# naturerobots/mesh_navigation

Hardware: AMD Instinct MI355X
Metric: plans/sec (Dijkstra makePlan device path incl. computeVectorMap, 1M-vertex mesh) (higher is better)
Workload: dtype f32

## Files before the change

### mesh_navigation_amd/csrc/mnav.hip

```cpp
#include <hip/hip_runtime.h>

#include <algorithm>
#include <array>
#include <atomic>
#include <chrono>
#include <cmath>
#include <cstdio>
#include <cstdlib>
#include <cstring>
#include <functional>
#include <map>
#include <string>
#include <vector>
#include <unordered_map>
#include <unistd.h>

#include "../../include/mnav.h"
#include "mnav_buf.h"
#include "mnav_build.h"
#include "mnav_eval.h"
#include "mnav_options.h"

using namespace mnav;

namespace {

#define MNAV_GLOBAL __attribute__((address_space(1)))
template <class T>
__device__ __forceinline__ MNAV_GLOBAL T* as_global(T* p) { return (MNAV_GLOBAL T*)p; }
template <class T>
__device__ __forceinline__ MNAV_GLOBAL T* as_global(const GPtr<T>& p) { return (MNAV_GLOBAL T*)p.p; }
typedef unsigned int u32x2 __attribute__((ext_vector_type(2)));
typedef unsigned int u32x4 __attribute__((ext_vector_type(4)));

constexpr int kBlock = 256;
constexpr int kChunk = 96;

#include "mnav_band.h"

#include "mnav_tiles.h"

#include "mnav_shard.h"

#include "mnav_finalize.h"

#include "mnav_plan_kernels.h"

#include "mnav_map_kernels.h"

}
#include "mnav_tb.h"
#include "mnav_tb_finalize.h"
#include "mnav_tbv.h"
#include "mnav_walk.h"
#include "mnav_obstacle.h"
#include "mnav_nbhd.h"
#include "mnav_clearance.h"
#include "mnav_locate.h"
#include "mnav_follow.h"
#include "mnav_rollout.h"
#include "mnav_replan.h"
#include "mnav_replan_each.h"
#include "mnav_tb_warm.h"
#include "mnav_graph.h"

struct WalkJob { const float* vecmap; float seed[3]; uint32_t seed_face; float target[3]; uint32_t target_face; };

__global__ __launch_bounds__(64) void k_backtrack(WalkMesh M, WalkInflation L, const WalkJob* __restrict__ jobs, double step_width, uint32_t cap,
                                                  float* __restrict__ pos_out, uint32_t* __restrict__ face_out, int32_t* __restrict__ ctl)
{
  __shared__ uint32_t list[kWalkScratchWords];
  const uint32_t j = blockIdx.x;
  const WalkJob J = jobs[j];
  if (!J.vecmap) { if (threadIdx.x == 0) { ctl[2 * j] = 0; ctl[2 * j + 1] = 0; } return; }
  WalkField Fd;
  Fd.vecmap = J.vecmap;
  for (int k = 0; k < 3; ++k) Fd.seed_vs[k] = M.faces[3 * (size_t)J.seed_face + k];
  uint32_t n = 0;
  const int st = walk_backtrack(M, Fd, L, w3(J.seed[0], J.seed[1], J.seed[2]), J.seed_face, w3(J.target[0], J.target[1], J.target[2]), J.target_face,
                                step_width, cap, pos_out + 3 * (size_t)cap * j, face_out + (size_t)cap * j, &n, list);
  ctl[2 * j] = st; ctl[2 * j + 1] = (int32_t)n;
}
#include "mnav_fleet.h"
#include "mnav_plans.h"
namespace {

struct Slot {
  DevBuf<float> dist, dirn, vecmap;
  DevBuf<PopKey> tkey;
  DevBuf<uint32_t> pred, cutf, stamp, dirty, list0, list1;
  DevBuf<uint32_t> wlist0, wlist1, wstamp;
  Ctl* ctl = nullptr;
  DevBuf<Cnt> cnt;
  bool cvp_ready = false, band_ready = false;
  DevBuf<uint32_t> tpend0, tpend1;
  DevBuf<float> tlast;
  TCtl* tctl = nullptr;
  DevBuf<TCnt> tcnt;
  bool tile_ready = false;
};

}

struct mnav_ctx {
  int device = 0;
  Stream stream;
  std::string err;
  std::atomic<int> cancel{ 0 };
  DevBuf<uint32_t> d_cancel;
  PinnedBuf<uint32_t> h_one;
  Stream cancel_stream;
  uint32_t V = 0, F = 0, E = 0;
  std::vector<float> h_xyz, h_cost;
  std::vector<uint32_t> h_row_ptr, h_nbr_u;
  TbState tb; tb::Args tb_args{};
  bool tb_args_valid = false;
  bool want_vec = false;
  bool resident_vecmap = false;
  std::vector<uint32_t> caller_slot;
  std::vector<uint32_t> h_faces;
  std::vector<uint32_t> h_vf_ptr, h_vf;
  DevBuf<uint32_t> d_faces, d_vf_ptr, d_vf; bool walk_mesh_valid = false;
  DevBuf<float> d_walk_pos; DevBuf<uint32_t> d_walk_face; size_t walk_cap = 0;
  Event ev_link[2];
  DevBuf<WalkJob> d_walk_jobs; DevBuf<int32_t> d_walk_ctl; uint32_t walk_jobs_cap = 0;
  std::vector<uint8_t> h_invalid;
  bool have_mesh = false, have_costs = false, have_normals = false;
  DevBuf<uint32_t> d_row_ptr, d_nbr_u, d_nbr_e, d_crn_ptr, d_edge_vtx;
  DevBuf<CornerIdx> d_crn_idx;
  DevBuf<uint32_t> d_crn_walk;
  DevBuf<float> d_xyz, d_nrm, d_cost, d_w, d_edge_dist;
  DevBuf<uint8_t> d_invalid;
  DevBuf<Nbr> d_nbr; double nbr_limit = NAN; bool nbr_valid = false;
  DevBuf<Corner> d_crn; DevBuf<uint8_t> d_blocked; double crn_limit = NAN; bool crn_valid = false;
  FaceCirculation circ;
  DevBuf<uint32_t> d_verify_any; uint32_t verify_sweeps_used = 0;
  bool cvp_verify = true;
  int walk_max = kKeyWalkMax, descend_max = kDescendWalkMax;
  std::vector<Slot> slots;
  DevBuf<Plan> d_plans; uint32_t plans_cap = 0;
  DevBuf<PlanResult> d_res; PinnedBuf<PlanResult> h_res;
  DevBuf<float*> d_vecptrs;
  DevBuf<uint32_t> d_paths; size_t paths_words = 0; uint32_t path_stride = 0;
  DevBuf<uint32_t> d_over; DevBuf<unsigned long long> d_over_off; DevBuf<uint32_t> d_over_cap;
  DevBuf<uint32_t> d_pack; PinnedBuf<uint32_t> h_pack; DevBuf<uint32_t> d_pack_meta; size_t pack_words = 0, pack_meta_n = 0;
  PinnedBuf<Ctl> h_ctl;
  uint32_t infl_exact_bands = 0;
  DevBuf<float> d_seed_pos; uint32_t seed_pos_cap = 1;
  std::map<uint64_t, GraphExec> graphs;
  int dij_engine = 3;
  int last_engine = 0;
  bool lazy_paths = false;
  bool allow_lazy_paths = true;
  uint32_t max_steps = 1u << 20;
  double max_wall_s = 120.0;
  uint32_t tile_size = 512;
  float rounds_band_mult = 4.0f;
  float tile_band_user = 0.f, tile_band_auto = 1.f;
  DevBuf<uint32_t> d_t_rptr;
  HostTiles tiles_meta;
  DevBuf<uint32_t> d_t_vptr, d_t_verts, d_t_hptr, d_t_halo_verts, d_t_halo_tile, d_t_eptr, d_t_src, d_vert_tile, d_mismatch;
  DevBuf<uint16_t> d_t_rowptr, d_t_col;
  DevBuf<float> d_t_tw; bool tw_valid = false; uint32_t t_nnz = 0;
  struct Shard {
    bool ready = false, active = false, finalized = false;
    uint32_t rank = 0, world = 1, t_lo = 0, t_hi = 0, n_iface = 0, rounds_per_exchange = 8, j = 0;
    uint32_t seed = 0, target = 0; double offset = 0.3; uint32_t goal_tie1 = 0;
    DevBuf<uint32_t> d_iface_vert, d_wake_ptr, d_wake_tile, d_changed, d_minpend;
    DevBuf<uint8_t> d_iface_owner;
    std::vector<uint32_t> iface_vert;
    bool partition = false; DevBuf<uint8_t> d_owned;
    DevBuf<uint32_t> d_walk; uint32_t walk_cap = 0;
    std::map<std::array<uint64_t, 3>, GraphExec> graphs;
  } shard;
  double edge_cost_factor = 0.0;
  struct Layer { DevBuf<float> cost; DevBuf<uint8_t> lethal; DevBuf<float> dist, vec; DevBuf<uint8_t> vstate;
                 bool ready = false, have_vec = false;
                 double inflation_radius = 0, inscribed_radius = 0, inscribed_value = 0, lethal_value = 0; };
  std::vector<Layer> layers;
  DevBuf<Corner> d_crn_infl; bool crn_infl_valid = false;
  DevBuf<uint8_t> d_infl_mask, d_zero_u8;
  DevBuf<float> d_infl_keyd;
  mnav_obs::Bvh obs;
  mnav_nb::State nbhd;
  mnav_clr::State clr;
  mnav_loc::State loc;
  mnav_fol::Staging stage;
  mnav_fol::State fol;
  mnav_fleet::State fleet;
  mnav_fleet::PlanState plans;
  DevBuf<float> d_fnrm; bool have_face_normals = false;
  mnav_rol::Dev rol;
  mnav_chg::Scratch chg;
  mnav_map::State map;
  uint32_t infl_steps = 0, infl_bands = 0; uint64_t infl_evals = 0; float infl_ms = 0.f, infl_ms_wave = 0.f;
  DevBuf<TilePlan> d_tplans; uint32_t tplans_cap = 0;
  PinnedBuf<TCtl> h_tctl;
  size_t tile_lds = 0, fin_lds = 0;
  bool use_graph = true;
  DevBuf<uint32_t> d_wide_prefix; DevBuf<WideSched> d_wide_sched; uint32_t wide_cap = 0;
  DevBuf<float> d_vec3;
  uint32_t wide_groups = 1; Stream stream_g[kWideGroupsMax]; Event ev_fork[kWideGroupsMax];
  uint32_t cvp_wide_min_batch = 32;
  float delta_user = 0.f, delta_auto = 0.f;
  Options opt;
  uint32_t max_steps_auto = 1u << 20;
  DevBuf<uint32_t> d_ring; uint32_t ring_cap = 0; size_t ring_words = 0; PinnedBuf<AsyncCtl> h_actl; DevBuf<uint32_t> d_parked; size_t parked_words = 0;
  struct Replan {
    DevBuf<uint32_t> log; uint32_t len = 0; bool all = false;
    std::vector<uint32_t> seeds, targets, caller_slot; double cost_limit = 1.0, offset = 0.0; bool have_call = false, usable = false;
    bool partial = false;
    bool finalized = false;
    bool slot0_taken = false;
    bool vec_resident = false;
    int each_engines = 0;
    struct Warm {
      DevBuf<uint32_t> d_level; DevBuf<const float*> d_dist; DevBuf<ReplanCnt> d_cnt; uint32_t cap = 0;
      uint32_t plans = 0, kernel = 0, iters = 0, fallback = 0; uint64_t woken = 0, words = 0; bool live = false;
      float ms_warm = 0.f, ms_engine = 0.f, ms_finalize = 0.f;
    } warm;
    DevBuf<uint32_t> d_level, d_old_target; DevBuf<float> d_cut; DevBuf<ReplanCnt> d_cnt; uint32_t cap = 0;
    Event ev[5]; bool have_ev = false;
    uint32_t reason = 0, stat_log_len = 0, tiles_woken = 0, rounds = 0; uint64_t kept = 0, rewound = 0; std::vector<float> levels;
    float ms_level = 0.f, ms_rewind = 0.f, ms_rounds = 0.f, ms_finalize = 0.f;
    struct Each {
      DevBuf<uint8_t> d_cls; DevBuf<float> d_ratio; DevBuf<uint32_t> d_lists, d_counts, d_level;
      DevBuf<Plan> d_plans; DevBuf<TilePlan> d_tplans; DevBuf<float*> d_vecptrs; DevBuf<ReplanCnt> d_cnt; DevBuf<TCtl> d_tctl; DevBuf<PlanResult> d_res;
      uint32_t cap = 0;
      Event ev[7]; bool have_ev = false;
      uint32_t reason = 0, whole_fresh = 0, log_len = 0, counts[3] = { 0, 0, 0 }, tiles_woken = 0, rounds = 0; int fresh_engine = -1;
      uint64_t kept = 0, rewound = 0; std::vector<uint8_t> cls; std::vector<float> levels;
      float ms_classify = 0.f, ms_rewind = 0.f, ms_rounds = 0.f, ms_finalize = 0.f, ms_fresh = 0.f;
    } each;
  } rp;
  uint32_t last_planner = 0, last_n = 0;
  std::vector<uint32_t> last_target; double last_offset = 0.0;
  mnav_stats stats{};
  uint64_t algo_bytes = 0;
  Event ev[8];
  Event evc[2];
  double ms_chunks = 0.0;
  DevBuf<Ctl> d_ctl_pool; uint32_t ctl_pool_cap = 0;
  DevBuf<TCtl> d_tctl_pool; uint32_t tctl_pool_cap = 0;
};

namespace {

#define MTRACE(msg) do { if (opt_on(ctx->opt.trace)) { fprintf(stderr, "[mnav] %9.3f ms %s:%d %s\n", 1e-3 * (double)std::chrono::duration_cast<std::chrono::microseconds>(std::chrono::steady_clock::now().time_since_epoch()).count(), __func__, __LINE__, msg); fflush(stderr); } } while (0)
#define HIPCHK(call)                                                                               \
  do {                                                                                             \
    hipError_t e_ = (call);                                                                        \
    if (e_ != hipSuccess) {                                                                        \
      ctx->err = std::string(#call) + ": " + hipGetErrorString(e_) + " (" __FILE_NAME__ ":" + std::to_string(__LINE__) + ")"; \
      return -1;                                                                                   \
    }                                                                                              \
  } while (0)

float ev_ms(hipEvent_t a, hipEvent_t b);

void drop_graphs(mnav_ctx* ctx)
{
  ctx->graphs.clear();
  ctx->shard.graphs.clear();
}

void apply_options(mnav_ctx* ctx)
{
  const Options& o = ctx->opt;
  ctx->use_graph = !opt_on(o.no_graph);
  if (opt_set(o.dijkstra_engine)) { const int e = (int)o.dijkstra_engine; ctx->dij_engine = (e == 0 || e == 1 || e == 5 || e == 6) ? e : 3; }
  else ctx->dij_engine = 3;
  ctx->max_steps = opt_u32(o.max_steps, ctx->max_steps_auto);
  ctx->max_wall_s = opt_set(o.max_wall_s) ? o.max_wall_s : 120.0;
  ctx->cvp_verify = !opt_set(o.cvp_verify) || o.cvp_verify != 0.0;
  ctx->walk_max = opt_set(o.key_walk_max) ? (int)o.key_walk_max : kKeyWalkMax;
  ctx->descend_max = opt_set(o.descend_walk_max) ? (int)o.descend_walk_max : kDescendWalkMax;
  ctx->allow_lazy_paths = !opt_set(o.lazy_paths) || o.lazy_paths != 0.0;
  ctx->tile_band_user = opt_set(o.tile_band) ? (float)o.tile_band : 0.f;
  ctx->rounds_band_mult = opt_set(o.rounds_band_mult) ? (float)o.rounds_band_mult : 4.0f;
}

int ensure_plan_tables(mnav_ctx* ctx, uint32_t n);

int ensure_slots(mnav_ctx* ctx, uint32_t n, bool cvp, bool band, bool vec)
{
  const size_t V = ctx->V ? ctx->V : 1;
  while (ctx->slots.size() < n) {
    Slot s;
    HIPCHK(s.dist.alloc(4 * V)); HIPCHK(s.pred.alloc(4 * V));
    HIPCHK(s.cnt.alloc(4 * sizeof(Cnt)));
    ctx->slots.push_back(std::move(s));
  }
  for (uint32_t i = 0; i < n; ++i) {
    Slot& s = ctx->slots[i];
    if (band && !s.band_ready) {
      HIPCHK(alloc_group(s.stamp, 4 * V, s.dirty, 4 * V, s.list0, 4 * V, s.list1, 4 * V, s.wlist0, 4 * V, s.wlist1, 4 * V, s.wstamp, 4 * V));
      s.band_ready = true;
    }
    if (vec && !s.vecmap) HIPCHK(s.vecmap.alloc(12 * V));
  }
  if (cvp)
    for (uint32_t i = 0; i < n; ++i) {
      Slot& s = ctx->slots[i];
      if (!s.cvp_ready) {
        HIPCHK(alloc_group(s.tkey, sizeof(PopKey) * V, s.dirn, 4 * V, s.cutf, 4 * V));
        s.cvp_ready = true;
      }
    }
  if (ctx->ctl_pool_cap < n) {
    HIPCHK(ctx->d_ctl_pool.alloc(2 * sizeof(Ctl) * n));
    ctx->ctl_pool_cap = n;
  }
  for (uint32_t i = 0; i < n; ++i) ctx->slots[i].ctl = ctx->d_ctl_pool + 2 * i;
  return ensure_plan_tables(ctx, n);
}

int ensure_plan_tables(mnav_ctx* ctx, uint32_t n)
{
  if (ctx->plans_cap < n) {
    ctx->d_plans.reset(); ctx->d_res.reset(); ctx->h_res.reset(); ctx->h_ctl.reset(); ctx->d_vecptrs.reset();
    drop_graphs(ctx);
    HIPCHK(ctx->d_plans.alloc(sizeof(Plan) * n));
    HIPCHK(ctx->d_res.alloc(sizeof(PlanResult) * n));
    HIPCHK(ctx->h_res.alloc(sizeof(PlanResult) * n));
    HIPCHK(ctx->h_ctl.alloc(sizeof(Ctl) * 2 * n));
    HIPCHK(ctx->d_vecptrs.alloc(sizeof(float*) * n));
    ctx->plans_cap = n;
  }
  return 0;
}

uint32_t default_path_stride(const mnav_ctx* ctx)
{
  const double s = 16.0 * std::sqrt((double)ctx->V) + 1024.0;
  return (uint32_t)std::min<double>(s, (double)(ctx->V ? ctx->V : 1));
}
int ensure_paths(mnav_ctx* ctx, uint32_t n, uint32_t stride)
{
  const size_t words = (size_t)n * (stride ? stride : 1);
  if (ctx->paths_words < words) {
    ctx->paths_words = 0;
    HIPCHK(ctx->d_paths.alloc(sizeof(uint32_t) * words));
    ctx->paths_words = words;
  }
  ctx->path_stride = stride;
  return 0;
}
int ensure_paths(mnav_ctx* ctx, uint32_t n) { return ensure_paths(ctx, n, default_path_stride(ctx)); }

uint32_t blocks_per_plan(const mnav_ctx* ctx)
{
  const double want = 4.0 * std::sqrt((double)ctx->V) / kGroupsPerWave;
  uint32_t g = (uint32_t)std::ceil(want);
  if (opt_set(ctx->opt.blocks_per_plan)) g = opt_u32(ctx->opt.blocks_per_plan, g);
  if (g < 4) g = 4;
  if (g > 4096) g = 4096;
  return g;
}

template <uint32_t PLANNER>
int launch_steps(mnav_ctx* ctx, uint32_t n, uint32_t G, int count, bool wide)
{
  const bool fork = wide && ctx->wide_groups > 1;
  if (fork) {
    HIPCHK(hipEventRecord(ctx->ev_fork[0], ctx->stream));
    for (uint32_t g = 1; g < ctx->wide_groups; ++g) HIPCHK(hipStreamWaitEvent(ctx->stream_g[g], ctx->ev_fork[0], 0));
  }
  for (int j = 0; j < count; ++j) {
    if (wide) {
      uint32_t off = 0, poff = 0;
      for (uint32_t g = 0; g < ctx->wide_groups; ++g) {
        const uint32_t ng = (n * (g + 1u)) / ctx->wide_groups - off;
        hipStream_t st = g == 0 ? ctx->stream : ctx->stream_g[g];
        if (ng) {
          hipLaunchKernelGGL(k_cvp_ctl, dim3(1), dim3(256), 0, st, ctx->d_plans + off, ng, j % 6, ctx->d_wide_prefix + poff, ctx->d_wide_sched + g);
          hipLaunchKernelGGL(k_step_wide, dim3(G), dim3(kWave), 0, st, ctx->d_plans + off, ng, j % 6, ctx->d_wide_prefix + poff, ctx->d_wide_sched + g);
          hipLaunchKernelGGL(k_step_repair, dim3(blocks_per_plan(ctx), kRepairRows), dim3(kWave), 0, st, ctx->d_plans + off, j % 6,
                             ctx->d_wide_prefix + poff + ng + 1u, ctx->d_wide_sched + g);
        }
        off += ng; poff += 2u * ng + 2u;
      }
    }
    else hipLaunchKernelGGL(k_step<PLANNER>, dim3(G, n), dim3(kWave), 0, ctx->stream, ctx->d_plans, j % 6);
  }
  if (fork) {
    for (uint32_t g = 1; g < ctx->wide_groups; ++g) {
      HIPCHK(hipEventRecord(ctx->ev_fork[g], ctx->stream_g[g]));
      HIPCHK(hipStreamWaitEvent(ctx->stream, ctx->ev_fork[g], 0));
    }
  }
  HIPCHK(hipGetLastError());
  return 0;
}

__global__ void k_stamp_to_host(unsigned long long* __restrict__ dst_host) { *dst_host = wall_clock64(); }

template <uint32_t PLANNER>
int run_chunk(mnav_ctx* ctx, uint32_t n, uint32_t G, bool wide)
{
  if (!ctx->use_graph) return launch_steps<PLANNER>(ctx, n, G, opt_set(ctx->opt.debug_chunk) ? (int)ctx->opt.debug_chunk : kChunk, wide);
  const uint64_t key = ((uint64_t)PLANNER << 60) | ((uint64_t)(wide ? ctx->wide_groups : 0u) << 57) | ((uint64_t)n << 32) | G;
  auto it = ctx->graphs.find(key);
  if (it == ctx->graphs.end()) {
    hipGraph_t g = nullptr;
    HIPCHK(hipStreamBeginCapture(ctx->stream, hipStreamCaptureModeThreadLocal));
    const int rc = launch_steps<PLANNER>(ctx, n, G, kChunk, wide);
    hipError_t e = hipStreamEndCapture(ctx->stream, &g);
    if (rc != 0 || e != hipSuccess) { ctx->err = "graph capture failed"; return -1; }
    GraphExec ge;
    HIPCHK(hipGraphInstantiate(ge.out(), g, nullptr, nullptr, 0));
    (void)hipGraphDestroy(g);
    it = ctx->graphs.emplace(key, std::move(ge)).first;
  }
  HIPCHK(hipGraphLaunch(it->second, ctx->stream));
  return 0;
}

int materialize(mnav_ctx* ctx, bool cvp, double cost_limit)
{
  const uint32_t V = ctx->V;
  const uint32_t gb = (V + kBlock - 1) / kBlock;
  if (!cvp) {
    if (ctx->nbr_valid && ctx->nbr_limit == cost_limit) return 0;
    if (!ctx->d_nbr) HIPCHK(ctx->d_nbr.alloc(sizeof(Nbr) * (size_t)(ctx->E ? 2 * (size_t)ctx->E : 1)));
    hipLaunchKernelGGL(k_build_nbr, dim3(gb ? gb : 1), dim3(kBlock), 0, ctx->stream, V, ctx->d_row_ptr, ctx->d_nbr_u,
                       ctx->d_nbr_e, ctx->d_w, ctx->d_cost, ctx->d_invalid, cost_limit, ctx->d_nbr);
    HIPCHK(hipGetLastError());
    ctx->nbr_limit = cost_limit; ctx->nbr_valid = true; ctx->tw_valid = false; ctx->tb.w_valid = false;
  } else {
    if (ctx->crn_valid && ctx->crn_limit == cost_limit) return 0;
    if (!ctx->d_crn) HIPCHK(ctx->d_crn.alloc(sizeof(Corner) * (size_t)(ctx->F ? 3 * (size_t)ctx->F : 1)));
    if (!ctx->d_blocked) HIPCHK(ctx->d_blocked.alloc(V ? V : 1));
    hipLaunchKernelGGL(k_build_crn, dim3(gb ? gb : 1), dim3(kBlock), 0, ctx->stream, V, ctx->d_crn_ptr, ctx->d_crn_idx,
                       ctx->d_w, ctx->d_cost, ctx->d_invalid, cost_limit, ctx->d_crn, ctx->d_blocked);
    HIPCHK(hipGetLastError());
    ctx->crn_limit = cost_limit; ctx->crn_valid = true;
  }
  return 0;
}

int verify_sweeps(mnav_ctx* ctx, uint32_t n)
{
  if (!ctx->d_verify_any) HIPCHK(ctx->d_verify_any.alloc(4));
  uint32_t gv = (ctx->V / kGroupsPerWave + 3) / 4;
  if (gv < 1) gv = 1;
  if (gv > 8192) gv = 8192;
  ctx->verify_sweeps_used = 0;
  for (int sweep = 0; sweep <= kVerifySweeps; ++sweep) {
// ... 557 lines not shown
}

static int layer_inflation_impl(mnav_ctx* ctx, uint32_t layer, uint32_t input_layer, double inflation_radius, double inscribed_radius,
                                double inscribed_value, double lethal_value, double cost_scaling_factor, const uint8_t* invalid,
                                const uint8_t* d_invalid, const mnav_map::Diff* diff)
{
  if (input_layer >= ctx->layers.size() || !ctx->layers[input_layer].ready) { ctx->err = "input layer is not resident"; return -1; }
  if (layer == input_layer) { ctx->err = "a layer cannot inflate itself"; return -1; }
  if (layer_slot(ctx, layer, true)) return -1;
  if (ctx->V > (1u << kKeyIdBits)) { ctx->err = "the ordered wave supports meshes of up to 2^26 vertices"; return -1; }
  if (ensure_edge_distances(ctx)) return -1;
  const uint32_t V = ctx->V;
  const uint32_t gb = (V + kBlock - 1) / kBlock ? (V + kBlock - 1) / kBlock : 1;
  if (!ctx->d_crn_infl) HIPCHK(ctx->d_crn_infl.alloc(sizeof(Corner) * (size_t)(ctx->F ? 3 * (size_t)ctx->F : 1)));
  if (!ctx->crn_infl_valid) {
    hipLaunchKernelGGL(k_build_crn_infl, dim3(gb), dim3(kBlock), 0, ctx->stream, V, ctx->d_crn_ptr, ctx->d_crn_idx, ctx->d_edge_dist, ctx->d_crn_infl);
    HIPCHK(hipGetLastError());
    ctx->crn_infl_valid = true;
  }
  const size_t Vn = V ? V : 1;
  if (!ctx->d_infl_mask) HIPCHK(ctx->d_infl_mask.alloc(Vn));
  if (!ctx->d_zero_u8) { HIPCHK(ctx->d_zero_u8.alloc(Vn)); HIPCHK(hipMemsetAsync(ctx->d_zero_u8, 0, Vn, ctx->stream)); }
  if (!ctx->d_infl_keyd) HIPCHK(ctx->d_infl_keyd.alloc(4 * Vn));
  DevBuf<uint8_t> d_inv;
  if (invalid) { HIPCHK(d_inv.alloc(Vn)); HIPCHK(hipMemcpyAsync(d_inv, invalid, V, hipMemcpyHostToDevice, ctx->stream)); d_invalid = d_inv; }
  mnav_ctx::Layer& L = ctx->layers[layer];
  mnav_ctx::Layer& In = ctx->layers[input_layer];
  L.inflation_radius = inflation_radius; L.inscribed_radius = inscribed_radius; L.inscribed_value = inscribed_value; L.lethal_value = lethal_value;
  hipLaunchKernelGGL(k_infl_mask, dim3(gb), dim3(kBlock), 0, ctx->stream, V, In.lethal, d_invalid, ctx->d_infl_mask);
  if (!diff) HIPCHK(hipMemcpyAsync(L.lethal, In.lethal, V, hipMemcpyDeviceToDevice, ctx->stream));
  if (ensure_slots(ctx, 1, true, true, false)) return -1;
  Slot& s = ctx->slots[0];
  ctx->caller_slot.assign(1, kNone);
  ctx->rp.slot0_taken = true;
  ctx->shard.finalized = false;
  Plan P;
  memset(&P, 0, sizeof(P));
  P.planner = kPlannerCvp; P.V = V;
  P.row_ptr = ctx->d_row_ptr.get(); P.nbr = nullptr; P.crn_ptr = ctx->d_crn_ptr.get(); P.crn = ctx->d_crn_infl.get(); P.blocked = ctx->d_zero_u8.get();
  P.dist = L.dist.get(); P.tkey = s.tkey.get(); P.pred = s.pred.get(); P.dirn = s.dirn.get(); P.cutf = s.cutf.get(); P.stamp = s.stamp.get(); P.dirty = s.dirty.get();
  P.list[0] = s.list0.get(); P.list[1] = s.list1.get(); P.wlist[0] = s.wlist0.get(); P.wlist[1] = s.wlist1.get(); P.wstamp = s.wstamp.get(); P.cap = V; P.ctl = s.ctl; P.cnt = s.cnt.get();
  const float maxd = (float)inflation_radius;
  P.delta = maxd > 0.f ? maxd : 1.0f;
  P.offset = 0.0; P.max_steps = ctx->max_steps; P.walk_max = ctx->walk_max; P.descend_max = ctx->descend_max;
  for (int k = 0; k < 3; ++k) { P.seed[k] = kNone; P.target[k] = kNone; P.seed_d[k] = 0.f; P.seed_expands[k] = 1; P.target_expands[k] = 0; }
  P.seed_face = kNone;
  P.seed_mask = ctx->d_infl_mask.get(); P.keyd = ctx->d_infl_keyd.get(); P.infl_max = maxd;
  HIPCHK(hipMemcpyAsync(ctx->d_plans, &P, sizeof(Plan), hipMemcpyHostToDevice, ctx->stream));
  HIPCHK(hipEventRecord(ctx->ev[1], ctx->stream));
  uint32_t gi = (V + kBlock * 4 - 1) / (kBlock * 4);
  if (gi < 1) gi = 1;
  if (gi > 4096) gi = 4096;
  hipLaunchKernelGGL(k_init<kPlannerCvp>, dim3(gi, 1), dim3(kBlock), 0, ctx->stream, ctx->d_plans);
  hipLaunchKernelGGL(k_infl_ctl, dim3(1), dim3(64), 0, ctx->stream, ctx->d_plans);
  hipLaunchKernelGGL(k_infl_seed, dim3(gi), dim3(kBlock), 0, ctx->stream, ctx->d_plans);
  HIPCHK(hipGetLastError());
  uint32_t G = blocks_per_plan(ctx) * 12u;
  if (G > 8192u) G = 8192u;
  const auto t_start = std::chrono::steady_clock::now();
  Ctl last{};
  ctx->infl_exact_bands = 0;
  for (;;) {
    if (std::chrono::duration<double>(std::chrono::steady_clock::now() - t_start).count() > ctx->max_wall_s) {
      ctx->err = "inflation wave exceeded the wall-clock guard"; return -1;
    }
    const auto t_c0 = std::chrono::steady_clock::now();
    const bool tr = opt_on(ctx->opt.trace);
    unsigned long long* const stamps = reinterpret_cast<unsigned long long*>(ctx->h_res.get());
    if (tr) { HIPCHK(hipEventRecord(ctx->ev[4], ctx->stream)); hipLaunchKernelGGL(k_stamp_to_host, dim3(1), dim3(1), 0, ctx->stream, stamps); }
    if (run_chunk<kPlannerCvp>(ctx, 1, G, false)) return -1;
    if (tr) HIPCHK(hipEventRecord(ctx->ev[5], ctx->stream));
    const auto t_c1 = std::chrono::steady_clock::now();
    if (tr) hipLaunchKernelGGL(k_stamp_to_host, dim3(1), dim3(1), 0, ctx->stream, stamps + 1);
    HIPCHK(hipMemcpyAsync(ctx->h_ctl, ctx->d_ctl_pool, 2 * sizeof(Ctl), hipMemcpyDeviceToHost, ctx->stream));
    HIPCHK(hipStreamSynchronize(ctx->stream));
    const auto t_c2 = std::chrono::steady_clock::now();
    float dev_ms = 0.f;
    if (tr) (void)hipEventElapsedTime(&dev_ms, ctx->ev[4], ctx->ev[5]);
    last = ctx->h_ctl[0].it > ctx->h_ctl[1].it ? ctx->h_ctl[0] : ctx->h_ctl[1];
    if (opt_on(ctx->opt.trace))
      fprintf(stderr, "[mnav] inflation it %d n %u thr %.6f fixed %.6f width %.4g bands %u band_steps %u shrinks %u cuts %u repair %u evals %u wread %u wbase %u done %u (verify sweeps of the previous wave %u) host ms: since start %.3f, this chunk's launch %.3f, its wait %.3f, the chunk on the device %.3f, by the device's own clock %.3f\n", last.it,
              last.n, last.thr, last.thr_fixed, last.width, last.bands, last.band_steps, last.shrinks, last.cuts, last.repair, last.evals, last.wread, last.wbase, last.done, ctx->verify_sweeps_used,
              1e3 * std::chrono::duration<double>(t_c0 - t_start).count(), 1e3 * std::chrono::duration<double>(t_c1 - t_c0).count(), 1e3 * std::chrono::duration<double>(t_c2 - t_c1).count(), dev_ms, tr ? (double)(stamps[1] - stamps[0]) * 1e-5 : 0.0);
    if (last.done) break;
    if (last.exact_wanted) {
      hipLaunchKernelGGL(k_exact_band, dim3(1), dim3(kWave), 0, ctx->stream, ctx->d_plans, (uint32_t*)nullptr);
      HIPCHK(hipGetLastError());
      ++ctx->infl_exact_bands;
    }
  }
  HIPCHK(hipEventRecord(ctx->ev[2], ctx->stream));
  if (verify_sweeps(ctx, 1)) return -1;
  if (diff) {
    using namespace mnav_map;
    const InflRule rule{ L.dist, In.lethal, inflation_radius, inscribed_radius, inscribed_value, lethal_value, cost_scaling_factor };
    const uint32_t nblk = blocks(V) ? blocks(V) : 1, fresh = L.ready ? 0u : 1u;
    hipLaunchKernelGGL(k_node_count<InflRule>, dim3(nblk), dim3(kChgBlock), 0, ctx->stream, V, rule, fresh, L.cost, L.lethal, diff->blk, nblk);
    hipLaunchKernelGGL(k_node_scan, dim3(1), dim3(kChgBlock), 0, ctx->stream, nblk, diff->blk, diff->cnt);
    hipLaunchKernelGGL(k_node_emit<InflRule>, dim3(nblk), dim3(kChgBlock), 0, ctx->stream, V, rule, fresh, L.cost, L.lethal, diff->blk, nblk, diff->ids);
  } else {
    hipLaunchKernelGGL(k_infl_cost, dim3(gb), dim3(kBlock), 0, ctx->stream, V, L.dist, inflation_radius, inscribed_radius, inscribed_value,
                       lethal_value, cost_scaling_factor, L.cost);
  }
  HIPCHK(hipGetLastError());
  L.have_vec = false;
  if (!L.vec) HIPCHK(L.vec.alloc(12 * Vn));
  if (!L.vstate) HIPCHK(L.vstate.alloc(3 * Vn));
  if (!ctx->d_verify_any) HIPCHK(ctx->d_verify_any.alloc(4));
  DevBuf<uint32_t> d_vctl;
  HIPCHK(d_vctl.alloc(16));
  HIPCHK(hipMemsetAsync(d_vctl, 0, 16, ctx->stream));
  uint8_t *st0 = L.vstate, *st1 = L.vstate + Vn, *acc = L.vstate + 2 * Vn;
  hipLaunchKernelGGL(k_infl_accum, dim3(gb), dim3(kBlock), 0, ctx->stream, ctx->d_plans, ctx->d_crn_walk, ctx->d_xyz, L.vec, st0, acc, d_vctl);
  uint32_t vctl[4] = { 0, 0, 0, 0 };
  bool vec_ok = true;
  for (int sweep = 0; sweep < 4096; ++sweep) {
    HIPCHK(hipMemsetAsync(d_vctl, 0, 8, ctx->stream));
    hipLaunchKernelGGL(k_infl_assign, dim3(gb), dim3(kBlock), 0, ctx->stream, ctx->d_plans, L.vec, st0, st1, acc, d_vctl);
    HIPCHK(hipMemcpyAsync(vctl, d_vctl, 16, hipMemcpyDeviceToHost, ctx->stream));
    HIPCHK(hipStreamSynchronize(ctx->stream));
    std::swap(st0, st1);
    if (vctl[2]) { vec_ok = false; break; }
    if (vctl[0] == 0) break;
    if (vctl[1] == 0) { vec_ok = false; break; }
  }
  if (st0 != L.vstate) HIPCHK(hipMemcpyAsync(L.vstate, st0, Vn, hipMemcpyDeviceToDevice, ctx->stream));
  d_vctl.reset();
  L.have_vec = vec_ok;
  HIPCHK(hipEventRecord(ctx->ev[3], ctx->stream));
  Cnt flags{};
  HIPCHK(hipMemcpyAsync(&flags, s.cnt + 3, sizeof(Cnt), hipMemcpyDeviceToHost, ctx->stream));
  if (diff) HIPCHK(hipMemcpyAsync(diff->h_cnt, diff->cnt, sizeof(uint32_t) * mnav_map::kCounters, hipMemcpyDeviceToHost, ctx->stream));
  HIPCHK(hipStreamSynchronize(ctx->stream));
  ctx->infl_steps = (uint32_t)(last.it < 0 ? 0 : last.it); ctx->infl_bands = last.bands; ctx->infl_evals = last.evals;
  ctx->infl_ms = ev_ms(ctx->ev[1], ctx->ev[3]); ctx->infl_ms_wave = ev_ms(ctx->ev[1], ctx->ev[2]);
  if (last.overflow) { ctx->err = "inflation wave did not converge (work-list overflow or step limit)"; return -1; }
  if (flags.n_next & kFlagWalkLimit) { ctx->err = "inflation wave: cascade-tree walk bound hit; the result may not be the reference's"; return -1; }
  if (flags.changed) { ctx->err = "inflation wave: the converged state is not a fixed point of the replay rule"; return -1; }
  L.ready = true;
  return 0;
}

int mnav_layer_inflation(mnav_ctx* ctx, uint32_t layer, uint32_t input_layer, double inflation_radius, double inscribed_radius,
                         double inscribed_value, double lethal_value, double cost_scaling_factor, const uint8_t* invalid)
{
  if (!ctx) return -1;
  ctx->err.clear();
  return layer_inflation_impl(ctx, layer, input_layer, inflation_radius, inscribed_radius, inscribed_value, lethal_value, cost_scaling_factor,
                              invalid, nullptr, nullptr);
}

int mnav_layer_download(mnav_ctx* ctx, uint32_t layer, float* costs_out, uint8_t* lethal_out, float* distances_out)
{
  if (!ctx) return -1;
  ctx->err.clear();
  if (layer >= ctx->layers.size() || !ctx->layers[layer].ready) { ctx->err = "layer is not resident"; return -1; }
  if (hipSetDevice(ctx->device) != hipSuccess) { ctx->err = "hipSetDevice failed"; return -1; }
  mnav_ctx::Layer& L = ctx->layers[layer];
  if (costs_out) HIPCHK(hipMemcpyAsync(costs_out, L.cost, sizeof(float) * ctx->V, hipMemcpyDeviceToHost, ctx->stream));
  if (lethal_out) HIPCHK(hipMemcpyAsync(lethal_out, L.lethal, ctx->V, hipMemcpyDeviceToHost, ctx->stream));
  if (distances_out) {
    if (!L.dist) { ctx->err = "this layer keeps no distances"; return -1; }
    HIPCHK(hipMemcpyAsync(distances_out, L.dist, sizeof(float) * ctx->V, hipMemcpyDeviceToHost, ctx->stream));
  }
  HIPCHK(hipStreamSynchronize(ctx->stream));
  return 0;
}

int mnav_layer_download_vectors(mnav_ctx* ctx, uint32_t layer, float* vectors_out, uint8_t* has_vector_out)
{
  if (!ctx) return -1;
  ctx->err.clear();
  if (layer >= ctx->layers.size() || !ctx->layers[layer].ready) { ctx->err = "layer is not resident"; return -1; }
  mnav_ctx::Layer& L = ctx->layers[layer];
  if (!L.have_vec) { ctx->err = "this layer has no vector field (not an inflation layer, or a vertex with more than 15 neighbours)"; return -1; }
  if (hipSetDevice(ctx->device) != hipSuccess) { ctx->err = "hipSetDevice failed"; return -1; }
  const uint32_t V = ctx->V;
  if (vectors_out) HIPCHK(hipMemcpyAsync(vectors_out, L.vec, 12 * (size_t)V, hipMemcpyDeviceToHost, ctx->stream));
  std::vector<uint8_t> st(V ? V : 1);
  if (has_vector_out) HIPCHK(hipMemcpyAsync(st.data(), L.vstate, V, hipMemcpyDeviceToHost, ctx->stream));
  HIPCHK(hipStreamSynchronize(ctx->stream));
  if (has_vector_out) for (uint32_t v = 0; v < V; ++v) has_vector_out[v] = st[v] == 1 ? 1 : 0;
  return 0;
}

int mnav_layer_stats(const mnav_ctx* ctx, uint32_t* steps, uint32_t* bands, uint64_t* evals, float* ms, uint32_t* verify_sweeps, float* ms_wave)
{
  if (!ctx) return -1;
  if (steps) *steps = ctx->infl_steps;
  if (bands) *bands = ctx->infl_bands;
  if (evals) *evals = ctx->infl_evals;
  if (ms) *ms = ctx->infl_ms;
  if (verify_sweeps) *verify_sweeps = ctx->verify_sweeps_used;
  if (ms_wave) *ms_wave = ctx->infl_ms_wave;
  return 0;
}

int mnav_combine_layers(mnav_ctx* ctx, int mode, uint32_t n_layers, const uint32_t* layers, const float* weights, double edge_cost_factor,
                        const uint8_t* invalid)
{
  if (!ctx) return -1;
  ctx->err.clear();
  if (!ctx->have_mesh) { ctx->err = "mnav_upload_mesh has not been called"; return -1; }
  if (mode != 0 && mode != 1) { ctx->err = "combination mode must be 0 (max) or 1 (weighted sum)"; return -1; }
  if ((n_layers && !layers) || (mode == 1 && n_layers && !weights) || n_layers > 64) { ctx->err = "bad layer list"; return -1; }
  if (hipSetDevice(ctx->device) != hipSuccess) { ctx->err = "hipSetDevice failed"; return -1; }
  std::vector<const float*> ptrs(n_layers ? n_layers : 1, nullptr);
  for (uint32_t l = 0; l < n_layers; ++l) {
    if (layers[l] >= ctx->layers.size() || !ctx->layers[layers[l]].ready) { ctx->err = "layer is not resident"; return -1; }
    ptrs[l] = ctx->layers[layers[l]].cost;
  }
  ctx->rp.all = true;
  if (ensure_edge_distances(ctx)) return -1;
  DevBuf<const float*> d_ptrs; DevBuf<float> d_wts;
  HIPCHK(d_ptrs.alloc(sizeof(float*) * (n_layers + 1)));
  HIPCHK(d_wts.alloc(sizeof(float) * (n_layers + 1)));
  int rc = 0;
  if (n_layers && hipMemcpyAsync(d_ptrs, ptrs.data(), sizeof(float*) * n_layers, hipMemcpyHostToDevice, ctx->stream) != hipSuccess) rc = -1;
  if (rc == 0 && mode == 1 && n_layers && hipMemcpyAsync(d_wts, weights, sizeof(float) * n_layers, hipMemcpyHostToDevice, ctx->stream) != hipSuccess) rc = -1;
  if (rc == 0 && ctx->d_cost.upload(ctx->stream, nullptr, ctx->V) != hipSuccess) { ctx->err = "cost buffer allocation failed"; rc = -1; }
  if (rc == 0) {
    const uint32_t gb = (ctx->V + kBlock - 1) / kBlock;
    hipLaunchKernelGGL(k_combine_resident, dim3(gb ? gb : 1), dim3(kBlock), 0, ctx->stream, ctx->V, mode, n_layers, d_ptrs, d_wts, ctx->d_cost);
    if (hipGetLastError() != hipSuccess) rc = -1;
  }
  if (rc != 0 && ctx->err.empty()) ctx->err = "layer combination failed";
  if (rc == 0) rc = edge_weight_pass(ctx, edge_cost_factor, invalid, nullptr, nullptr);
  (void)hipStreamSynchronize(ctx->stream);
  return rc;
}

int mnav_combine_layers_update(mnav_ctx* ctx, int mode, uint32_t n_layers, const uint32_t* layers, const float* weights, uint32_t n,
                               const uint32_t* vertex_ids)
{
  if (!ctx) return -1;
  ctx->err.clear();
  if (!ctx->have_costs) { ctx->err = "no combined costs resident yet (mnav_combine_layers first)"; return -1; }
  if (mode != 0 && mode != 1) { ctx->err = "combination mode must be 0 (max) or 1 (weighted sum)"; return -1; }
  if ((n_layers && !layers) || (mode == 1 && n_layers && !weights) || n_layers > 64) { ctx->err = "bad layer list"; return -1; }
  if (n == 0) return 0;
  if (!vertex_ids) { ctx->err = "null id array"; return -1; }
  for (uint32_t i = 0; i < n; ++i) if (vertex_ids[i] >= ctx->V) { ctx->err = "vertex id out of range"; return -1; }
  if (hipSetDevice(ctx->device) != hipSuccess) { ctx->err = "hipSetDevice failed"; return -1; }
  std::vector<const float*> ptrs(n_layers ? n_layers : 1, nullptr);
  for (uint32_t l = 0; l < n_layers; ++l) {
    if (layers[l] >= ctx->layers.size() || !ctx->layers[layers[l]].ready) { ctx->err = "layer is not resident"; return -1; }
    ptrs[l] = ctx->layers[layers[l]].cost;
  }
  ctx->rp.all = true;
  DevBuf<const float*> d_ptrs; DevBuf<float> d_wts, d_vals; DevBuf<uint32_t> d_ids;
  HIPCHK(d_ptrs.alloc(sizeof(float*) * (n_layers + 1)));
  HIPCHK(d_wts.alloc(sizeof(float) * (n_layers + 1)));
  HIPCHK(d_vals.alloc(sizeof(float) * n));
  HIPCHK(d_ids.alloc(sizeof(uint32_t) * n));
  std::vector<float> vals(n);
  int rc = 0;
  if (n_layers && hipMemcpyAsync(d_ptrs, ptrs.data(), sizeof(float*) * n_layers, hipMemcpyHostToDevice, ctx->stream) != hipSuccess) rc = -1;
  if (rc == 0 && mode == 1 && n_layers && hipMemcpyAsync(d_wts, weights, sizeof(float) * n_layers, hipMemcpyHostToDevice, ctx->stream) != hipSuccess) rc = -1;
  if (rc == 0 && hipMemcpyAsync(d_ids, vertex_ids, sizeof(uint32_t) * n, hipMemcpyHostToDevice, ctx->stream) != hipSuccess) rc = -1;
  if (rc == 0) {
    hipLaunchKernelGGL(k_combine_resident_ids, dim3((n + kBlock - 1) / kBlock), dim3(kBlock), 0, ctx->stream, n, d_ids, mode, n_layers, d_ptrs, d_wts,
                       ctx->d_cost, d_vals);
    if (ctx->edge_cost_factor != 0.0)
      hipLaunchKernelGGL(k_update_edge_weights, dim3((8 * n + kBlock - 1) / kBlock), dim3(kBlock), 0, ctx->stream, n, d_ids, ctx->d_row_ptr,
                         ctx->d_nbr_u, ctx->d_nbr_e, ctx->d_edge_dist, ctx->d_cost, ctx->edge_cost_factor, ctx->d_w);
    if (hipGetLastError() != hipSuccess) rc = -1;
  }
  if (rc == 0 && hipMemcpyAsync(vals.data(), d_vals, sizeof(float) * n, hipMemcpyDeviceToHost, ctx->stream) != hipSuccess) rc = -1;
  (void)hipStreamSynchronize(ctx->stream);
  if (rc != 0) { if (ctx->err.empty()) ctx->err = "incremental combination failed"; return rc; }
  for (uint32_t i = 0; i < n; ++i) ctx->h_cost[vertex_ids[i]] = vals[i];
  ctx->nbr_valid = ctx->crn_valid = false;
  return 0;
}

struct TailSub { const Plan* plans; PlanResult* res; float* const* vecptrs; uint32_t n_vec; const uint32_t* slot; };
static int dijkstra_tail(mnav_ctx* ctx, uint32_t m, int engine, const std::vector<uint32_t>& map, std::vector<uint32_t>& codes, float* dist_out,
                         uint32_t* pred_out, uint32_t* path_out, uint32_t path_cap, uint32_t* path_len, float* vecmap_out, bool want_vecmap,
                         const TailSub* sub = nullptr)
{
  const uint32_t V = ctx->V;
  const Plan* const d_plans = sub ? sub->plans : ctx->d_plans.get();
  PlanResult* const d_res = sub ? sub->res : ctx->d_res.get();
  const uint32_t n_vec = sub ? sub->n_vec : m;
  const PathRows rows1{ ctx->d_paths, ctx->path_stride, nullptr, nullptr };
  PathRows rows2{ nullptr, 0u, nullptr, nullptr };
  const uint32_t gc = (V + kBlock * 4 - 1) / (kBlock * 4);
  if (engine == 5 && ctx->lazy_paths) {
    hipLaunchKernelGGL(k_tb_path, dim3(m), dim3(kWave), 0, ctx->stream, ctx->tb_args, ctx->d_row_ptr, ctx->d_nbr, V, ctx->d_res, rows1, ctx->d_mismatch);
    ctx->tb.count_pending = true;
  } else if (ctx->lazy_paths) {
    hipLaunchKernelGGL(k_path_lazy, dim3(m), dim3(kWave), 0, ctx->stream, ctx->d_plans, ctx->d_tplans, ctx->d_res, rows1, ctx->d_mismatch);
    hipLaunchKernelGGL(k_count_goal, dim3(gc ? gc : 1, m), dim3(kBlock), 0, ctx->stream, ctx->d_plans, ctx->d_res);
  } else
  hipLaunchKernelGGL(k_finish<kPlannerDijkstra>, dim3(m), dim3(64), 0, ctx->stream, d_plans, d_res, rows1);
  if (engine == 1)
    hipLaunchKernelGGL(k_count, dim3(gc ? gc : 1, m), dim3(kBlock), 0, ctx->stream, d_plans, d_res);
  if (sub && m > n_vec)
    hipLaunchKernelGGL(k_count, dim3(gc ? gc : 1, m - n_vec), dim3(kBlock), 0, ctx->stream, d_plans + n_vec, d_res + n_vec);
  (void)hipEventRecord(ctx->ev[4], ctx->stream);
  if (want_vecmap && n_vec && !(engine == 5 && !ctx->lazy_paths))
    hipLaunchKernelGGL(k_vecmap_dijkstra, dim3(gc ? gc : 1, n_vec), dim3(kBlock), 0, ctx->stream, d_plans, ctx->d_xyz, sub ? sub->vecptrs : ctx->d_vecptrs.get());
  (void)hipEventRecord(ctx->ev[5], ctx->stream);
  if (hipMemcpyAsync(ctx->h_res, d_res, sizeof(PlanResult) * m, hipMemcpyDeviceToHost, ctx->stream) != hipSuccess ||
      hipStreamSynchronize(ctx->stream) != hipSuccess) { ctx->err = "result download failed"; return -1; }
  {
    size_t over_words = 0;
    std::vector<unsigned long long> ooff(m, 0ull); std::vector<uint32_t> ocap(m, 0u);
    for (uint32_t k = 0; k < m; ++k)
      if (ctx->h_res[k].code == kPathOverflow) { ooff[k] = over_words; ocap[k] = ctx->h_res[k].path_len; over_words += ctx->h_res[k].path_len; }
    if (over_words) {
      std::vector<PlanResult> keep(ctx->h_res.get(), ctx->h_res + m);
      ctx->d_over.reset(); ctx->d_over_off.reset(); ctx->d_over_cap.reset();
      if (ctx->d_over.alloc(4 * over_words) != hipSuccess || ctx->d_over_off.alloc(8 * (size_t)m) != hipSuccess || ctx->d_over_cap.alloc(4 * (size_t)m) != hipSuccess ||
          hipMemcpyAsync(ctx->d_over_off, ooff.data(), 8 * (size_t)m, hipMemcpyHostToDevice, ctx->stream) != hipSuccess ||
          hipMemcpyAsync(ctx->d_over_cap, ocap.data(), 4 * (size_t)m, hipMemcpyHostToDevice, ctx->stream) != hipSuccess)
        { ctx->err = "path buffers: out of memory"; return -1; }
      rows2 = PathRows{ ctx->d_over, 0u, ctx->d_over_off, ctx->d_over_cap };
      if (engine == 5 && ctx->lazy_paths) hipLaunchKernelGGL(k_tb_path, dim3(m), dim3(kWave), 0, ctx->stream, ctx->tb_args, ctx->d_row_ptr, ctx->d_nbr, V, ctx->d_res, rows2, ctx->d_mismatch);
      else if (ctx->lazy_paths) hipLaunchKernelGGL(k_path_lazy, dim3(m), dim3(kWave), 0, ctx->stream, ctx->d_plans, ctx->d_tplans, ctx->d_res, rows2, ctx->d_mismatch);
      else hipLaunchKernelGGL(k_finish<kPlannerDijkstra>, dim3(m), dim3(64), 0, ctx->stream, d_plans, d_res, rows2);
      if (hipMemcpyAsync(ctx->h_res, d_res, sizeof(PlanResult) * m, hipMemcpyDeviceToHost, ctx->stream) != hipSuccess ||
          hipStreamSynchronize(ctx->stream) != hipSuccess) { ctx->err = "result download failed"; return -1; }
      for (uint32_t k = 0; k < m; ++k) ctx->h_res[k].settled = keep[k].settled;
    }
  }
  if (ctx->last_engine != 1) {
    uint32_t mism = 0;
    if (hipMemcpy(&mism, ctx->d_mismatch, 4, hipMemcpyDeviceToHost) != hipSuccess || mism != 0) {
      ctx->err = "tiled SSSP did not reach its fixed point (" + std::to_string(mism) + " vertices)";
      return -1;
    }
  }
  MTRACE("results downloaded");
  std::vector<uint32_t> offs(m + 1, 0), lens(m, 0);
  for (uint32_t k = 0; k < m; ++k) {
    lens[k] = (ctx->h_res[k].code == MNAV_SUCCESS) ? ctx->h_res[k].path_len : 0u;
    offs[k + 1] = offs[k] + lens[k];
  }
  const size_t total = offs[m];
  if (total && path_out && path_cap) {
    if (ctx->pack_words < total) {
      ctx->d_pack.reset(); ctx->h_pack.reset(); ctx->pack_words = 0;
      const size_t want = total + total / 4 + 1024;
      if (ctx->d_pack.alloc(4 * want) != hipSuccess || ctx->h_pack.alloc(4 * want) != hipSuccess)
        { ctx->err = "path buffers: out of memory"; return -1; }
      ctx->pack_words = want;
    }
    if (ctx->pack_meta_n < 2 * (size_t)m) {
      ctx->pack_meta_n = 0;
      if (ctx->d_pack_meta.alloc(4 * 2 * (size_t)m) != hipSuccess) { ctx->err = "path buffers: out of memory"; return -1; }
      ctx->pack_meta_n = 2 * (size_t)m;
    }
    if (hipMemcpyAsync(ctx->d_pack_meta, offs.data(), 4 * (size_t)m, hipMemcpyHostToDevice, ctx->stream) != hipSuccess ||
        hipMemcpyAsync(ctx->d_pack_meta + m, lens.data(), 4 * (size_t)m, hipMemcpyHostToDevice, ctx->stream) != hipSuccess)
      { ctx->err = "path download failed"; return -1; }
    hipLaunchKernelGGL(k_pack_paths, dim3(m), dim3(kBlock), 0, ctx->stream, rows1, rows2, ctx->d_pack_meta, ctx->d_pack_meta + m, ctx->d_pack);
    if (hipMemcpyAsync(ctx->h_pack, ctx->d_pack, 4 * total, hipMemcpyDeviceToHost, ctx->stream) != hipSuccess ||
        hipStreamSynchronize(ctx->stream) != hipSuccess) { ctx->err = "path download failed"; return -1; }
  }
  MTRACE("paths downloaded");
  for (uint32_t k = 0; k < m; ++k) {
    const uint32_t i = map[k];
    const PlanResult& r = ctx->h_res[k];
    const Slot& sl = ctx->slots[sub ? sub->slot[k] : k];
    codes[i] = r.code;
    if (r.code == MNAV_SUCCESS) {
      if (path_len) path_len[i] = r.path_len;
      if (path_out && path_cap && r.path_len)
        memcpy(path_out + (size_t)i * path_cap, ctx->h_pack + offs[k], 4 * (size_t)std::min(r.path_len, path_cap));
    }
    if (dist_out && hipMemcpyAsync(dist_out + (size_t)i * V, sl.dist, 4 * (size_t)V, hipMemcpyDeviceToHost, ctx->stream) != hipSuccess)
      { ctx->err = "dist download failed"; return -1; }
    if (pred_out && hipMemcpyAsync(pred_out + (size_t)i * V, sl.pred, 4 * (size_t)V, hipMemcpyDeviceToHost, ctx->stream) != hipSuccess)
      { ctx->err = "pred download failed"; return -1; }
    if (vecmap_out && want_vecmap && hipMemcpyAsync(vecmap_out + (size_t)i * 3 * V, sl.vecmap, 12 * (size_t)V, hipMemcpyDeviceToHost, ctx->stream) != hipSuccess)
      { ctx->err = "vecmap download failed"; return -1; }
  }
  MTRACE("paths copied out");
  (void)hipEventRecord(ctx->ev[6], ctx->stream);
  if (hipStreamSynchronize(ctx->stream) != hipSuccess) { ctx->err = "sync failed"; return -1; }
  if (engine == 5 && tb_clean_other(ctx)) return -1;
  finish_stats(ctx, m, false);
  MTRACE("stats done");
  return 0;
}

static int dijkstra_auto_engine(mnav_ctx* ctx, uint32_t m0)
{
  const double tiles = std::max(1.0, (double)ctx->V / (0.9 * ctx->tb.T));
  const bool fills = m0 >= ctx->tb.min_batch && m0 <= 65535u && (double)m0 >= tiles / 1000.0;
  return (m0 <= opt_u32(ctx->opt.async_max_batch, 160u)) ? 6 : fills ? 5 : 0;
}

static int dijkstra_order(mnav_ctx* ctx, int engine, std::vector<PlanIn>& in, std::vector<uint32_t>& map)
{
  const uint32_t V = ctx->V;
  if (engine == 5 && in.size() > 1) {
    if (tb_build(ctx)) return -1;
    std::vector<uint32_t> ord(in.size());
    std::iota(ord.begin(), ord.end(), 0u);
    const std::vector<uint32_t>& vt = ctx->tb.vert_tile;
    std::stable_sort(ord.begin(), ord.end(), [&](uint32_t x, uint32_t y) { return vt[in[x].seed[0]] < vt[in[y].seed[0]]; });
    std::vector<PlanIn> in2(in.size()); std::vector<uint32_t> map2(in.size());
    for (size_t i = 0; i < in.size(); ++i) { in2[i] = in[ord[i]]; map2[i] = map[ord[i]]; }
    in.swap(in2); map.swap(map2);
  } else
  if (in.size() > 1 && ctx->h_xyz.size() == 3 * (size_t)V) {
    std::vector<uint32_t> ord(in.size());
    std::iota(ord.begin(), ord.end(), 0u);
    std::vector<float> est(in.size());
    for (size_t i = 0; i < in.size(); ++i) {
      const float* a = &ctx->h_xyz[3 * (size_t)in[i].seed[0]];
      const float* b = &ctx->h_xyz[3 * (size_t)in[i].target[0]];
      est[i] = (a[0] - b[0]) * (a[0] - b[0]) + (a[1] - b[1]) * (a[1] - b[1]) + (a[2] - b[2]) * (a[2] - b[2]);
    }
    std::stable_sort(ord.begin(), ord.end(), [&](uint32_t x, uint32_t y) { return est[x] > est[y]; });
    std::vector<PlanIn> in2(in.size()); std::vector<uint32_t> map2(in.size());
    for (size_t i = 0; i < in.size(); ++i) { in2[i] = in[ord[i]]; map2[i] = map[ord[i]]; }
    in.swap(in2); map.swap(map2);
  }
  return 0;
}

static int dijkstra_dispatch(mnav_ctx* ctx, uint32_t m, const std::vector<PlanIn>& in, double offset, bool engine_auto, int* engine_io)
{
  int engine = *engine_io;
  const bool want_path = true;
  int rc = (engine == 0) ? run_dijkstra_tiled(ctx, m, in, offset)
         : (engine == 6) ? run_dijkstra_async(ctx, m, in, offset)
         : (engine == 5) ? run_dijkstra_tb(ctx, m, in, offset)
                         : run_plans<kPlannerDijkstra>(ctx, m, in, offset, want_path);
  if (engine == 6 && (rc == 2 || (rc == 3 && engine_auto))) { ctx->err.clear(); engine = 0; rc = run_dijkstra_tiled(ctx, m, in, offset); }
  if (rc == 3) rc = -1;
  MTRACE("engine returned");
  if (rc != 0) (void)hipStreamSynchronize(ctx->stream);
  *engine_io = engine;
  return rc;
}

static uint32_t dijkstra_impl(mnav_ctx* ctx, uint32_t n, const uint32_t* seeds, const uint32_t* targets, double offset,
                              double cost_limit, uint32_t* codes_out, float* dist_out, uint32_t* pred_out, uint32_t* path_out,
                              uint32_t path_cap, uint32_t* path_len, float* vecmap_out, bool want_vecmap)
{
  if (check_ready(ctx)) return MNAV_INTERNAL_ERROR;
  ctx->err.clear();
  if (offset != offset) { ctx->err = "goal_dist_offset is NaN"; return MNAV_INTERNAL_ERROR; }
  ctx->cancel.store(0);
  if (ctx->d_cancel) { (void)hipStreamSynchronize(ctx->cancel_stream); (void)hipMemsetAsync(ctx->d_cancel, 0, 4, ctx->stream); }
  want_vecmap = want_vecmap || ctx->resident_vecmap;
  ctx->want_vec = want_vecmap;
  if (hipSetDevice(ctx->device) != hipSuccess) { ctx->err = "hipSetDevice failed"; return MNAV_INTERNAL_ERROR; }
  MTRACE("start");
  const uint32_t V = ctx->V;
  uint32_t worst = MNAV_SUCCESS;
  {
    mnav_ctx::Replan& R = ctx->rp;
    const std::vector<uint32_t> s_(seeds, seeds + n), t_(targets, targets + n);
    R.seeds = s_; R.targets = t_; R.cost_limit = cost_limit; R.offset = offset; R.have_call = true; R.usable = false; R.partial = false;
    R.finalized = false; R.each_engines = 0; R.warm.live = false;
  }
  std::vector<PlanIn> in; std::vector<uint32_t> map;
  std::vector<uint32_t> codes(n, MNAV_SUCCESS);
  std::vector<uint8_t> cleared(n, 0);
  for (uint32_t i = 0; i < n; ++i) {
    if (path_len) path_len[i] = 0;
    if (seeds[i] >= V) { codes[i] = MNAV_INVALID_START; continue; }
    if (targets[i] >= V) { codes[i] = MNAV_INVALID_GOAL; continue; }
    if (seeds[i] == targets[i]) { cleared[i] = 1; continue; }
    PlanIn p{};
    for (int k = 0; k < 3; ++k) { p.seed[k] = kNone; p.target[k] = kNone; p.seed_d[k] = 0.f; p.seed_expands[k] = 1; p.target_expands[k] = 1; }
    p.seed[0] = seeds[i]; p.target[0] = targets[i]; p.seed_face = kNone;
    in.push_back(p); map.push_back(i);
  }
  int engine = ctx->dij_engine;
  const bool engine_auto = engine == 3;
  ctx->lazy_paths = ctx->allow_lazy_paths && !dist_out && !pred_out && !want_vecmap && !ctx->resident_vecmap;
  {
    const uint32_t m0 = (uint32_t)in.size();
    if (engine == 3) engine = dijkstra_auto_engine(ctx, m0);
    if (engine == 5 && m0 > 65535u) engine = 0;
    if (engine == 1 && offset < 0.0) engine = 0;
  }
  if (dijkstra_order(ctx, engine, in, map)) return MNAV_INTERNAL_ERROR;
  ctx->caller_slot.assign(n, kNone);
  ctx->shard.finalized = false;
  for (size_t i = 0; i < map.size(); ++i) ctx->caller_slot[map[i]] = (uint32_t)i;
  (void)hipEventRecord(ctx->ev[0], ctx->stream);
  const uint32_t m = (uint32_t)in.size();
  ctx->tb.count_pending = false; ctx->tb_args_valid = false;
  ctx->last_planner = kPlannerDijkstra; ctx->last_n = 0;
  ctx->last_target.resize(m); for (uint32_t k = 0; k < m; ++k) ctx->last_target[k] = in[k].target[0];
  ctx->last_offset = offset;
  if (m) {
    if (materialize(ctx, false, cost_limit)) return MNAV_INTERNAL_ERROR;
    const int rc = dijkstra_dispatch(ctx, m, in, offset, engine_auto, &engine);
    if (rc < 0) return MNAV_INTERNAL_ERROR;
    if (rc == 1) { for (uint32_t i = 0; i < n; ++i) if (codes_out) codes_out[i] = MNAV_CANCELED; return MNAV_CANCELED; }
    ctx->last_engine = engine; ctx->last_n = m;
    if (engine == 1) ctx->lazy_paths = false;
    if (dijkstra_tail(ctx, m, engine, map, codes, dist_out, pred_out, path_out, path_cap, path_len, vecmap_out, want_vecmap)) return MNAV_INTERNAL_ERROR;
    ctx->rp.usable = engine == 0 || engine == 6 || (engine == 5 && !ctx->lazy_paths);
    ctx->rp.finalized = !ctx->lazy_paths;
    ctx->rp.vec_resident = want_vecmap;
  }
  ctx->rp.slot0_taken = false; ctx->rp.each_engines = 0; ctx->rp.warm.live = false;
  ctx->rp.caller_slot = ctx->caller_slot; ctx->rp.len = 0; ctx->rp.all = false;
  ctx->rp.partial = m != n;
  for (uint32_t i = 0; i < n; ++i) {
    if (codes[i] == MNAV_INVALID_START || codes[i] == MNAV_INVALID_GOAL || cleared[i]) {
      if (dist_out) for (uint32_t v = 0; v < V; ++v) dist_out[(size_t)i * V + v] = INFINITY;
      if (pred_out) for (uint32_t v = 0; v < V; ++v) pred_out[(size_t)i * V + v] = v;
    }
    if (codes_out) codes_out[i] = codes[i];
    if (codes[i] != MNAV_SUCCESS && worst == MNAV_SUCCESS) worst = codes[i];
  }
  return worst;
}

uint32_t mnav_plan_dijkstra(mnav_ctx* ctx, uint32_t seed_vertex, uint32_t target_vertex, double goal_dist_offset, double cost_limit,
                            float* dist_out, uint32_t* pred_out, uint32_t* path_out, uint32_t path_cap, uint32_t* path_len,
                            float* vecmap_out)
{
  if (!ctx) return MNAV_INTERNAL_ERROR;
  uint32_t code = MNAV_INTERNAL_ERROR;
  uint32_t len = 0;
  const uint32_t rc = dijkstra_impl(ctx, 1, &seed_vertex, &target_vertex, goal_dist_offset, cost_limit, &code, dist_out, pred_out,
                                    path_out, path_cap, &len, vecmap_out, true);
  if (path_len) *path_len = len;
  return rc == MNAV_INTERNAL_ERROR || rc == MNAV_CANCELED ? rc : code;
}

uint32_t mnav_plan_dijkstra_batch(mnav_ctx* ctx, uint32_t n, const uint32_t* seeds, const uint32_t* targets, double goal_dist_offset,
                                  double cost_limit, uint32_t* codes_out, float* dist_out, uint32_t* pred_out, uint32_t* path_out,
                                  uint32_t path_cap, uint32_t* path_len)
{
  if (!ctx) return MNAV_INTERNAL_ERROR;
  if (n == 0) return MNAV_SUCCESS;
  if (!seeds || !targets) { ctx->err = "null seeds/targets"; return MNAV_INTERNAL_ERROR; }
  return dijkstra_impl(ctx, n, seeds, targets, goal_dist_offset, cost_limit, codes_out, dist_out, pred_out, path_out, path_cap,
                       path_len, nullptr, false);
}

static uint32_t cvp_impl(mnav_ctx* ctx, uint32_t n, const float* seed_pos, const uint32_t* seed_faces, const uint32_t* target_faces,
                         double goal_dist_offset, double cost_limit, uint32_t* codes_out, float* dist_out, uint32_t* pred_out,
                         float* direction_out, uint32_t* cutface_out, float* vecmap_out)
{
  if (check_ready(ctx)) return MNAV_INTERNAL_ERROR;
  ctx->err.clear();
  if (goal_dist_offset != goal_dist_offset) { ctx->err = "goal_dist_offset is NaN"; return MNAV_INTERNAL_ERROR; }
  ctx->cancel.store(0);
  if (ctx->d_cancel) { (void)hipStreamSynchronize(ctx->cancel_stream); (void)hipMemsetAsync(ctx->d_cancel, 0, 4, ctx->stream); }
  if (hipSetDevice(ctx->device) != hipSuccess) { ctx->err = "hipSetDevice failed"; return MNAV_INTERNAL_ERROR; }
  const uint32_t V = ctx->V;
  if (!ctx->have_normals) { ctx->err = "vertex normals were not uploaded"; return MNAV_INTERNAL_ERROR; }
  if (V > (1u << kKeyIdBits)) { ctx->err = "CVP pop keys hold 26-bit vertex ids: mesh too large"; return MNAV_INTERNAL_ERROR; }
  std::vector<uint32_t> codes(n, MNAV_SUCCESS), map;
  std::vector<PlanIn> in;
  std::vector<float> sp;
  for (uint32_t i = 0; i < n; ++i) {
    if (seed_faces[i] >= ctx->F) { codes[i] = MNAV_INVALID_START; continue; }
    if (target_faces[i] >= ctx->F) { codes[i] = MNAV_INVALID_GOAL; continue; }
    PlanIn p{};
    for (int k = 0; k < 3; ++k) {
      p.seed[k] = ctx->h_faces[3 * (size_t)seed_faces[i] + k];
      p.target[k] = ctx->h_faces[3 * (size_t)target_faces[i] + k];
    }
    for (int k = 0; k < 3; ++k) {
      const float dx = seed_pos[3 * (size_t)i] - ctx->h_xyz[3 * (size_t)p.seed[k]];
      const float dy = seed_pos[3 * (size_t)i + 1] - ctx->h_xyz[3 * (size_t)p.seed[k] + 1];
      const float dz = seed_pos[3 * (size_t)i + 2] - ctx->h_xyz[3 * (size_t)p.seed[k] + 2];
      const float l2 = dx * dx + dy * dy + dz * dz;
      p.seed_d[k] = sqrtf(l2);
      p.seed_expands[k] = (!((double)ctx->h_cost[p.seed[k]] >= cost_limit) && !ctx->h_invalid[p.seed[k]]) ? 1u : 0u;
      p.target_expands[k] = (!((double)ctx->h_cost[p.target[k]] >= cost_limit) && !ctx->h_invalid[p.target[k]]) ? 1u : 0u;
    }
    p.seed_face = seed_faces[i];
    in.push_back(p); map.push_back(i);
    sp.insert(sp.end(), seed_pos + 3 * (size_t)i, seed_pos + 3 * (size_t)i + 3);
  }
  const uint32_t m = (uint32_t)in.size();
  ctx->caller_slot.assign(n, kNone);
  ctx->shard.finalized = false;
  for (size_t i = 0; i < map.size(); ++i) ctx->caller_slot[map[i]] = (uint32_t)i;
  (void)hipEventRecord(ctx->ev[0], ctx->stream);
  ctx->tb.count_pending = false; ctx->tb_args_valid = false;
  ctx->last_planner = kPlannerCvp; ctx->last_n = 0; ctx->last_engine = 1; ctx->rp.warm.live = false;
  ctx->rp.usable = ctx->rp.partial = false;
  uint32_t worst = MNAV_SUCCESS;
  if (m) {
    if (materialize(ctx, true, cost_limit)) return MNAV_INTERNAL_ERROR;
    if (ctx->seed_pos_cap < m) {
      if (ctx->d_seed_pos.alloc(12 * (size_t)m) != hipSuccess) { ctx->err = "alloc failed"; return MNAV_INTERNAL_ERROR; }
      ctx->seed_pos_cap = m;
    }
    if (hipMemcpyAsync(ctx->d_seed_pos, sp.data(), 12 * (size_t)m, hipMemcpyHostToDevice, ctx->stream) != hipSuccess)
      { ctx->err = "seed upload failed"; return MNAV_INTERNAL_ERROR; }
    const int rc = run_plans<kPlannerCvp>(ctx, m, in, goal_dist_offset, false);
    if (rc != 0) (void)hipStreamSynchronize(ctx->stream);
    if (rc < 0) return MNAV_INTERNAL_ERROR;
    if (rc == 1) { if (codes_out) for (uint32_t i = 0; i < n; ++i) codes_out[i] = MNAV_CANCELED; return MNAV_CANCELED; }
    ctx->last_n = m;
    hipLaunchKernelGGL(k_finish<kPlannerCvp>, dim3(m), dim3(64), 0, ctx->stream, ctx->d_plans, ctx->d_res, PathRows{ nullptr, 0u, nullptr, nullptr });
    const uint32_t gc = (V + kBlock * 4 - 1) / (kBlock * 4);
    hipLaunchKernelGGL(k_count, dim3(gc ? gc : 1, m), dim3(kBlock), 0, ctx->stream, ctx->d_plans, ctx->d_res);
    (void)hipEventRecord(ctx->ev[4], ctx->stream);
    hipLaunchKernelGGL(k_vecmap_cvp, dim3(gc ? gc : 1, m), dim3(kBlock), 0, ctx->stream, ctx->d_plans, ctx->d_xyz, ctx->d_nrm,
                       ctx->d_vecptrs, ctx->d_seed_pos);
    (void)hipEventRecord(ctx->ev[5], ctx->stream);
    bool ok = hipMemcpyAsync(ctx->h_res, ctx->d_res, sizeof(PlanResult) * m, hipMemcpyDeviceToHost, ctx->stream) == hipSuccess;
    for (uint32_t k = 0; k < m && ok; ++k) {
      const uint32_t i = map[k];
      Slot& s = ctx->slots[k];
      if (ok && dist_out) ok = hipMemcpyAsync(dist_out + (size_t)i * V, s.dist, 4 * (size_t)V, hipMemcpyDeviceToHost, ctx->stream) == hipSuccess;
      if (ok && pred_out) ok = hipMemcpyAsync(pred_out + (size_t)i * V, s.pred, 4 * (size_t)V, hipMemcpyDeviceToHost, ctx->stream) == hipSuccess;
      if (ok && direction_out) ok = hipMemcpyAsync(direction_out + (size_t)i * V, s.dirn, 4 * (size_t)V, hipMemcpyDeviceToHost, ctx->stream) == hipSuccess;
      if (ok && cutface_out) ok = hipMemcpyAsync(cutface_out + (size_t)i * V, s.cutf, 4 * (size_t)V, hipMemcpyDeviceToHost, ctx->stream) == hipSuccess;
      if (ok && vecmap_out) ok = hipMemcpyAsync(vecmap_out + (size_t)i * 3 * V, s.vecmap, 12 * (size_t)V, hipMemcpyDeviceToHost, ctx->stream) == hipSuccess;
    }
    (void)hipEventRecord(ctx->ev[6], ctx->stream);
    if (!ok || hipStreamSynchronize(ctx->stream) != hipSuccess) { ctx->err = "output download failed"; return MNAV_INTERNAL_ERROR; }
    finish_stats(ctx, m, true);
    for (uint32_t k = 0; k < m; ++k) {
      codes[map[k]] = ctx->h_res[k].code;
      if (ctx->h_res[k].code == MNAV_INTERNAL_ERROR) {
        const uint32_t o = ctx->h_res[k].overflow;
        ctx->err = (o & 8u) ? "CVP: a walk over the cascade tree hit its bound on the converged state (pop order not guaranteed)"
                 : (o & 16u) ? "CVP: verification sweep found a vertex that is not a fixed point of the gather rule"
                             : "CVP wavefront did not converge (step cap)";
      }
    }
  }
  for (uint32_t i = 0; i < n; ++i) {
    if (codes_out) codes_out[i] = codes[i];
    if (codes[i] != MNAV_SUCCESS && worst == MNAV_SUCCESS) worst = codes[i];
  }
  return worst;
}

uint32_t mnav_plan_cvp(mnav_ctx* ctx, const float seed_pos[3], uint32_t seed_face, uint32_t target_face, double goal_dist_offset,
                       double cost_limit, float* dist_out, uint32_t* pred_out, float* direction_out, uint32_t* cutface_out,
                       float* vecmap_out)
{
  if (!ctx) return MNAV_INTERNAL_ERROR;
  if (!seed_pos) return MNAV_INVALID_START;
  uint32_t code = MNAV_INTERNAL_ERROR;
  const uint32_t rc = cvp_impl(ctx, 1, seed_pos, &seed_face, &target_face, goal_dist_offset, cost_limit, &code, dist_out, pred_out,
                               direction_out, cutface_out, vecmap_out);
  return (rc == MNAV_INTERNAL_ERROR || rc == MNAV_CANCELED) ? rc : code;
}

uint32_t mnav_plan_cvp_batch(mnav_ctx* ctx, uint32_t n, const float* seed_pos, const uint32_t* seed_faces, const uint32_t* target_faces,
                             double goal_dist_offset, double cost_limit, uint32_t* codes_out, float* dist_out, uint32_t* pred_out,
                             float* vecmap_out)
{
  if (!ctx) return MNAV_INTERNAL_ERROR;
  if (n == 0) return MNAV_SUCCESS;
  if (!seed_pos || !seed_faces || !target_faces) { ctx->err = "null seeds/targets"; return MNAV_INTERNAL_ERROR; }
  return cvp_impl(ctx, n, seed_pos, seed_faces, target_faces, goal_dist_offset, cost_limit, codes_out, dist_out, pred_out, nullptr, nullptr,
                  vecmap_out);
}

#include "mnav_shard_capi.h"
// ... 294 lines not shown
```

### mesh_navigation_amd/csrc/mnav_plan_kernels.h

```cpp
#pragma once

template <uint32_t PLANNER>
__global__ __launch_bounds__(kBlock) void k_init(const Plan* __restrict__ plans)
{
  const Plan& P = plans[blockIdx.y];
  const uint32_t stride = gridDim.x * kBlock;
  for (uint32_t v = blockIdx.x * kBlock + threadIdx.x; v < P.V; v += stride) {
    P.dist[v] = inf_f();
    P.pred[v] = v;
    if (P.stamp) { P.stamp[v] = 0u; P.dirty[v] = 0u; P.wstamp[v] = 0u; }
    if (PLANNER == kPlannerCvp) { P.tkey[v] = key_inf(); P.dirn[v] = 0.0f; P.cutf[v] = kNone; if (P.keyd) P.keyd[v] = inf_f(); }
  }
}

template <uint32_t PLANNER>
__global__ void k_seed(const Plan* __restrict__ plans)
{
  const Plan& P = plans[blockIdx.x];
  if (threadIdx.x != 0) return;
  constexpr int ns = (PLANNER == kPlannerCvp) ? 3 : 1;
  float m0 = inf_f();
  for (int k = 0; k < ns; ++k) {
    const uint32_t s = P.seed[k];
    P.dist[s] = P.seed_d[k];
    if (PLANNER == kPlannerCvp) { P.tkey[s] = make_key(P.seed_d[k], s); P.cutf[s] = P.seed_face; }
    m0 = fminf(m0, P.seed_d[k]);
  }
  uint32_t n = 0;
  uint32_t* l0 = P.list[0];
  for (int k = 0; k < ns; ++k) {
    const uint32_t s = P.seed[k];
    if (PLANNER == kPlannerCvp) {
      for (uint32_t i = P.crn_ptr[s]; i < P.crn_ptr[s + 1]; ++i) {
        const Corner c = P.crn[i];
        if (c.v1 == kNone) continue;
        if (P.stamp[c.v1] != 0xFFFFFFFFu) { P.stamp[c.v1] = 0xFFFFFFFFu; if (n < P.cap) l0[n] = c.v1; ++n; }
        if (P.stamp[c.v2] != 0xFFFFFFFFu) { P.stamp[c.v2] = 0xFFFFFFFFu; if (n < P.cap) l0[n] = c.v2; ++n; }
      }
    } else {
      for (uint32_t i = P.row_ptr[s]; i < P.row_ptr[s + 1]; ++i) {
        const uint32_t u = P.nbr[i].u;
        if (P.stamp[u] != 0xFFFFFFFFu) { P.stamp[u] = 0xFFFFFFFFu; if (n < P.cap) l0[n] = u; ++n; }
      }
    }
  }
  Ctl c0; memset(&c0, 0, sizeof(c0));
  c0.it = -1; c0.n = 0; c0.thr_fixed = -inf_f(); c0.goal_dist = inf_f(); c0.arm_vertex = kNone;
  c0.thr = m0 + P.delta; if (!(c0.thr > m0)) c0.thr = next_up(m0);
  for (int k = 0; k < ns; ++k) if (!(P.seed_d[k] < c0.thr)) c0.thr = next_up(P.seed_d[k]);
  c0.band_new = 1; c0.width = P.delta; c0.wmin = inf_f(); c0.epoch = 1;
  P.ctl[1] = c0;
  P.ctl[0] = c0;
  Cnt ci; memset(&ci, 0, sizeof(ci)); ci.n_next = n; ci.changed = 1; ci.minkey = 0x7f800000u; ci.minchg = 0x7f800000u;
  P.cnt[2] = ci;
  Cnt z; memset(&z, 0, sizeof(z)); z.minkey = 0x7f800000u; z.minchg = 0x7f800000u;
  P.cnt[0] = z; P.cnt[1] = z; P.cnt[3] = z;
}


constexpr uint32_t kPathOverflow = 0xFFFFFFF0u;
struct PathRows {
  uint32_t* base; uint32_t stride;
  const unsigned long long* off; const uint32_t* cap;
  __device__ __forceinline__ uint32_t* row(uint32_t k) const { return base + (off ? (size_t)off[k] : (size_t)k * stride); }
  __device__ __forceinline__ uint32_t capacity(uint32_t k) const { return cap ? cap[k] : stride; }
  __device__ __forceinline__ bool skip(uint32_t k) const { return cap && cap[k] == 0u; }
};

template <uint32_t PLANNER>
__global__ void k_finish(const Plan* __restrict__ plans, PlanResult* __restrict__ res, PathRows rows)
{
  const Plan& P = plans[blockIdx.x];
  if (threadIdx.x != 0 || rows.skip(blockIdx.x)) return;
  PlanResult& R = res[blockIdx.x];
  const Ctl a = P.ctl[0], b = P.ctl[1];
  const Ctl last = (a.it > b.it) ? a : b;
  R.steps = (uint32_t)(last.it < 0 ? 0 : last.it);
  R.bands = last.bands; R.armed = last.armed; R.overflow = last.overflow; R.goal_dist = last.goal_dist; R.shrinks = last.shrinks | (last.cuts << 16);
  R.evals = last.evals;
  R.path_len = 0;
  uint32_t code = kSuccess;
  if (PLANNER == kPlannerCvp) {
    if (P.cnt[3].n_next & kFlagWalkLimit) R.overflow |= 8u;
    if (P.cnt[3].changed) R.overflow |= 16u;
  }
  if (R.overflow || !last.done) code = kInternalError;
  else if (PLANNER == kPlannerDijkstra) {
    const uint32_t seed = P.seed[0], target = P.target[0];
    if (P.pred[target] == target) code = kNoPathFound;
    else {
      uint32_t* path = rows.row(blockIdx.x);
      const uint32_t cap = rows.capacity(blockIdx.x);
      uint32_t n = 0, v = target;
      while (v != seed && n <= P.V) { v = P.pred[v]; if (n < cap) path[n] = v; ++n; }
      if (v != seed) code = kInternalError;
      else if (n > cap) code = kPathOverflow;
      R.path_len = n;
    }
  } else {
    bool any = false;
    for (int k = 0; k < 3; ++k) any = any || (P.pred[P.target[k]] != P.target[k]);
    if (!any && !(P.target[0] == P.seed[0] && P.target[1] == P.seed[1] && P.target[2] == P.seed[2]))
      code = kNoPathFound;
  }
  R.code = code;
}

__global__ __launch_bounds__(kWave) void k_path_lazy(const Plan* __restrict__ plans, const TilePlan* __restrict__ tplans, PlanResult* __restrict__ res,
                                                     PathRows rows, uint32_t* __restrict__ mismatch)
{
  if (rows.skip(blockIdx.x)) return;
  const Plan& P = plans[blockIdx.x];
  const TilePlan& T = tplans[blockIdx.x];
  const int lane = threadIdx.x;
  PlanResult& R = res[blockIdx.x];
  const TCtl a = T.ctl[0], b = T.ctl[1];
  const TCtl last = (a.it > b.it) ? a : b;
  const uint32_t seed = P.seed[0], target = P.target[0];
  const float dt = P.dist[target];
  const GoalCut gcut = goal_cut(dt, P.offset, target);
  const float goal_dist = gcut.goal;
  uint32_t code = kSuccess, n = 0, bad = 0;
  if (last.pad[0] || !last.done) code = kInternalError;
  else if (!(dt < inf_f())) code = kNoPathFound;
  else {
    uint32_t* path = rows.row(blockIdx.x);
    const uint32_t cap = rows.capacity(blockIdx.x);
    uint32_t v = target;
    while (v != seed && n <= P.V) {
      const float dv = P.dist[v];
      float best_s = inf_f(), best_du = inf_f();
      uint32_t best_u = v;
      const uint32_t beg = P.row_ptr[v], end = P.row_ptr[v + 1];
      for (uint32_t i = beg + lane; i < end; i += kWave) {
        const Nbr nb = P.nbr[i];
        const float du = P.dist[nb.u];
        if (!expanded_source(gcut, du, nb.u)) continue;
        const float sm = du + nb.w;
        if (sm < best_s || (sm == best_s && sm < inf_f() && (du < best_du || (du == best_du && nb.u < best_u)))) { best_s = sm; best_du = du; best_u = nb.u; }
      }
#pragma unroll
      for (int o = 1; o < kWave; o <<= 1) {
        const float os = __shfl_xor(best_s, o), odu = __shfl_xor(best_du, o);
        const uint32_t ou = __shfl_xor(best_u, o);
        if (os < best_s || (os == best_s && os < inf_f() && (odu < best_du || (odu == best_du && ou < best_u)))) { best_s = os; best_du = odu; best_u = ou; }
      }
      if (f2u(best_s) != f2u(dv) || best_u == v) { bad = 1; break; }
      v = best_u;
      if (lane == 0 && n < cap) path[n] = v;
      ++n;
    }
    if (bad || v != seed) code = kInternalError;
    else if (n > cap) code = kPathOverflow;
  }
  if (lane == 0) {
    R.code = code; R.path_len = (code == kSuccess || code == kPathOverflow) ? n : 0;
    R.steps = (uint32_t)(last.it < 0 ? 0 : last.it); R.bands = last.sweeps; R.armed = (dt < inf_f()) ? 1u : 0u; R.overflow = last.pad[0];
    R.goal_dist = goal_dist; R.evals = last.acts; R.shrinks = 0;
    if (bad) atomicAdd(mismatch, 1u);
  }
}

__global__ __launch_bounds__(kBlock) void k_pack_paths(PathRows rows, PathRows over, const uint32_t* __restrict__ offs,
                                                       const uint32_t* __restrict__ lens, uint32_t* __restrict__ out)
{
  const uint32_t k = blockIdx.x, len = lens[k];
  const uint32_t* src = (over.cap && over.cap[k]) ? over.row(k) : rows.row(k);
  uint32_t* dst = out + offs[k];
  for (uint32_t q = threadIdx.x; q < len; q += kBlock) dst[q] = src[len - 1 - q];
}

__global__ __launch_bounds__(kBlock) void k_count_goal(const Plan* __restrict__ plans, PlanResult* __restrict__ res)
{
  const Plan& P = plans[blockIdx.y];
  const float dt = P.dist[P.target[0]];
  const float goal_dist = goal_cut(dt, P.offset, P.target[0]).cut;
  uint32_t c = 0;
  const uint32_t stride = gridDim.x * kBlock;
  for (uint32_t v = blockIdx.x * kBlock + threadIdx.x; v < P.V; v += stride) { const float d = P.dist[v]; c += (d < inf_f() && d <= goal_dist) ? 1u : 0u; }
  c = wave_sum(c);
  __shared__ uint32_t s_c[kBlock / 64];
  if ((threadIdx.x & 63) == 0) s_c[threadIdx.x >> 6] = c;
  __syncthreads();
  if (threadIdx.x == 0) {
    uint32_t tot = 0;
    for (int k = 0; k < kBlock / 64; ++k) tot += s_c[k];
    if (tot) atomicAdd(&res[blockIdx.y].settled, (unsigned long long)tot);
  }
}

__global__ __launch_bounds__(kBlock) void k_count(const Plan* __restrict__ plans, PlanResult* __restrict__ res)
{
  const Plan& P = plans[blockIdx.y];
  uint32_t c = 0;
  const uint32_t stride = gridDim.x * kBlock;
  for (uint32_t v = blockIdx.x * kBlock + threadIdx.x; v < P.V; v += stride) c += (P.dist[v] < inf_f()) ? 1u : 0u;
  c = wave_sum(c);
  __shared__ uint32_t s_c[kBlock / 64];
  if ((threadIdx.x & 63) == 0) s_c[threadIdx.x >> 6] = c;
  __syncthreads();
  if (threadIdx.x == 0) {
    uint32_t tot = 0;
    for (int k = 0; k < kBlock / 64; ++k) tot += s_c[k];
    if (tot) atomicAdd(&res[blockIdx.y].settled, (unsigned long long)tot);
  }
}
```

### mesh_navigation_amd/csrc/mnav_tb.h

```cpp
#pragma once

#include "mnav_tb_build.h"

namespace {

namespace tb {

#define MNAV_CONST __attribute__((address_space(4)))
typedef uint32_t u32x16 __attribute__((ext_vector_type(16)));
typedef const MNAV_CONST u32x16* cblk8_t;
typedef __attribute__((address_space(3))) uint32_t* lds_u32_t;
enum { kTwSoff = 0, kTwSl = 1, kTwNv = 2, kTwNh = 3, kTwSweepOff = 4, kTwSweepChunks = 5, kTwPreOff = 6, kTwPreChunks = 7,
       kTwPostOff = 8, kTwPostChunks = 9, kTwExpOff = 10, kTwExpN = 11 };
static_assert(offsetof(TbTile, exp_n) == 4 * kTwExpN && offsetof(TbTile, sweep_off) == 4 * kTwSweepOff, "TbTile layout");

struct Ctl {
  uint32_t n_cand[2];
  uint32_t n_items, next_item;
  uint32_t err;
  uint32_t iters;
  unsigned long long acts;
  unsigned long long sweeps;
  unsigned long long items;
  unsigned long long wakes;
  uint32_t n_pairs, pad_;
};

struct Args {
  const TbTile* tiles; const uint32_t* stream; const TbExp* exps;
  float* D; uint32_t* pend; uint32_t NP, ntiles;
  uint16_t* bucket; uint32_t* bcnt; uint2* items; Ctl* ctl;
  uint32_t* marr[2];
  float* thr; float* bnd;
  const uint32_t* seed; const uint32_t* target;
  const uint2* vaddr; const uint32_t* vert_tile;
  double offset; float band;
  uint8_t* pflag; uint32_t nblk;
  uint32_t* pairs; uint32_t n_flag16;
  uint32_t nblk_magic, nblk_shift;
  unsigned long long* wstat; uint32_t wstat_slots;
  uint32_t item_plans;
};

__device__ __forceinline__ size_t slot_addr(const uint2 va, uint32_t NP, uint32_t p)
{
  return (size_t)va.x * NP + (size_t)p * (va.y >> 8) + (va.y & 255u);
}

__device__ __forceinline__ uint32_t ldsr(uint32_t off) { return *(lds_u32_t)(uintptr_t)off; }
__device__ __forceinline__ void ldsw(uint32_t off, uint32_t v) { *(lds_u32_t)(uintptr_t)off = v; }
typedef __attribute__((address_space(3))) u32x4* lds_u32x4_t;
__device__ __forceinline__ u32x4 ldsr4(uint32_t off) { return *(lds_u32x4_t)(uintptr_t)off; }

__device__ __forceinline__ uint32_t rfl(uint32_t x) { return (uint32_t)__builtin_amdgcn_readfirstlane((int)x); }

__device__ __forceinline__ uint32_t div_by_magic(uint32_t n, uint32_t d, uint32_t magic, uint32_t shift)
{
  return d <= 1u ? n : (__umulhi(n, magic) >> shift);
}

}

__global__ __launch_bounds__(kBlock) void k_tb_weights(size_t n, const uint32_t* __restrict__ wsrc, const Nbr* __restrict__ nbr, uint32_t* __restrict__ stream)
{
  const size_t stride = (size_t)gridDim.x * kBlock;
  for (size_t i = (size_t)blockIdx.x * kBlock + threadIdx.x; i < n; i += stride) {
    const uint32_t s = wsrc[i];
    if (s != kNone) stream[i] = f2u(nbr[s].w);
  }
}

__global__ __launch_bounds__(kBlock) void k_tb_fill(u32x4* __restrict__ p, size_t n16, uint32_t v)
{
  const size_t stride = (size_t)gridDim.x * kBlock;
  const u32x4 x = { v, v, v, v };
  for (size_t i = (size_t)blockIdx.x * kBlock + threadIdx.x; i < n16; i += stride) __builtin_nontemporal_store(x, p + i);
}

__global__ __launch_bounds__(kBlock) void k_tb_seed(tb::Args A)
{
  const uint32_t p = blockIdx.x * kBlock + threadIdx.x;
  if (p >= A.NP) return;
  const uint32_t s = A.seed[p];
  const uint2 va = A.vaddr[s];
  A.D[tb::slot_addr(va, A.NP, p)] = 0.0f;
  const uint32_t t = A.vert_tile[s];
  const TbTile W = A.tiles[t];
  const uint32_t row = (va.y & 255u) * 256u;
  for (uint32_t k = 0; k < W.exp_n; ++k) {
    const TbExp e = A.exps[W.exp_off + k];
    if (e.u == row) A.D[(size_t)e.soff * A.NP + (size_t)p * e.sl + e.off] = 0.0f;
  }
  A.pend[(size_t)t * A.NP + p] = 0u;
  A.pflag[(size_t)t * A.nblk + (p >> 6)] = 1;
  A.marr[0][p] = 0u;
  A.ctl->n_cand[0] = 1u;
}

__global__ __launch_bounds__(kBlock) void k_tb_plan(tb::Args A, int par)
{
  const uint32_t p = blockIdx.x * kBlock + threadIdx.x;
  if (p == 0) { A.ctl->n_cand[par ^ 1] = 0u; A.ctl->next_item = 0u; A.ctl->n_items = 0u; A.ctl->n_pairs = 0u; A.ctl->iters += 1u; }
  if (p >= A.NP) return;
  const uint32_t mb = A.marr[par][p];
  A.marr[par ^ 1][p] = kTbInfBits;
  const float m = u2f(mb);
  const float dt = A.D[tb::slot_addr(A.vaddr[A.target[p]], A.NP, p)];
  const float bound = (float)((double)dt + fmax(A.offset, 0.0));
  const bool done = !(m < inf_f()) || m > bound;
  float thr = m + A.band;
  if (!(thr > m)) thr = next_up(m);
  A.thr[p] = done ? 0.0f : thr;
  A.bnd[p] = bound;
}

constexpr uint32_t kTbPairUnits = 4;
__global__ __launch_bounds__(kBlock) void k_tb_pairs(tb::Args A)
{
  __shared__ uint32_t s_wave[kBlock / 64], s_base;
  const int lane = threadIdx.x & 63, wave = threadIdx.x >> 6;
  const uint32_t i0 = (blockIdx.x * kBlock + threadIdx.x) * kTbPairUnits;
  u32x4 f[kTbPairUnits];
  uint32_t c = 0;
#pragma unroll
  for (uint32_t u = 0; u < kTbPairUnits; ++u) {
    f[u] = u32x4{ 0u, 0u, 0u, 0u };
    if (i0 + u < A.n_flag16) f[u] = ((MNAV_GLOBAL const u32x4*)as_global(A.pflag))[i0 + u];
    const uint32_t w[4] = { f[u].x, f[u].y, f[u].z, f[u].w };
#pragma unroll
    for (int k = 0; k < 4; ++k)
#pragma unroll
      for (int b = 0; b < 4; ++b) c += ((w[k] >> (8 * b)) & 0xFFu) ? 1u : 0u;
  }
  uint32_t incl = c;
#pragma unroll
  for (int o = 1; o < 64; o <<= 1) { const uint32_t x = __shfl_up(incl, o); if (lane >= o) incl += x; }
  if (lane == 63) s_wave[wave] = incl;
  __syncthreads();
  if (threadIdx.x == 0) {
    uint32_t tot = 0;
#pragma unroll
    for (int w = 0; w < kBlock / 64; ++w) { const uint32_t x = s_wave[w]; s_wave[w] = tot; tot += x; }
    s_base = tot ? atomicAdd(&A.ctl->n_pairs, tot) : 0u;
  }
  __syncthreads();
  uint32_t base = s_base + s_wave[wave] + incl - c;
  if (c) {
#pragma unroll
    for (uint32_t u = 0; u < kTbPairUnits; ++u) {
      const uint32_t w[4] = { f[u].x, f[u].y, f[u].z, f[u].w };
#pragma unroll
      for (int k = 0; k < 4; ++k)
#pragma unroll
        for (int b = 0; b < 4; ++b)
          if ((w[k] >> (8 * b)) & 0xFFu) A.pairs[base++] = 16u * (i0 + u) + 4u * k + b;
    }
  }
}

constexpr uint32_t kTbStatSlots = 16384;
constexpr uint32_t kTbScanWaves = 8192;
__global__ __launch_bounds__(kBlock) void k_tb_scan(tb::Args A, int par)
{
  const int lane = threadIdx.x & 63;
  const uint32_t wave = blockIdx.x * (kBlock / 64) + (threadIdx.x >> 6), nwaves = gridDim.x * (kBlock / 64);
  const uint32_t n_pairs = A.ctl->n_pairs;
  if (wave >= n_pairs) return;
  MNAV_GLOBAL const uint32_t* const pairs = as_global(A.pairs);
  MNAV_GLOBAL const float* const g_thr = as_global(A.thr);
  MNAV_GLOBAL const float* const g_bnd = as_global(A.bnd);
  MNAV_GLOBAL uint32_t* const g_pend = as_global(A.pend);
  MNAV_GLOBAL uint32_t* const g_min = as_global(A.marr[par ^ 1]);
  uint32_t carried = 0;
  struct Row { uint32_t pr, t, p, pb, pm; float thr, bnd; bool live; };
  auto fetch = [&](uint32_t pr, bool have) {
    Row r; r.pr = pr;
    const uint32_t t = tb::div_by_magic(pr, A.nblk, A.nblk_magic, A.nblk_shift), p = (pr - t * A.nblk) * 64u + (uint32_t)lane;
    r.live = have && t < A.ntiles && p < A.NP;
    r.t = r.live ? t : 0u; r.p = r.live ? p : 0u;
    r.pb = g_pend[(size_t)r.t * A.NP + r.p]; r.thr = g_thr[r.p]; r.bnd = g_bnd[r.p]; r.pm = g_min[r.p];
    return r;
  };
  uint32_t k = wave;
  const uint32_t last = n_pairs - 1u;
  uint32_t pr_next = pairs[min(k + nwaves, last)];
  Row cur = fetch(pairs[k], true);
  for (; k < n_pairs; k += nwaves) {
    asm volatile("" :: "v"(cur.pb), "v"(cur.thr), "v"(cur.bnd), "v"(cur.pm));
    const uint32_t t = cur.t, p = cur.p, pb = cur.pb;
    MNAV_GLOBAL uint32_t* const pe = g_pend + ((size_t)t * A.NP + p);
    bool ready = false, keep = false;
    if (cur.live && pb != kTbInfBits) {
      const float pv = u2f(pb);
      if (pv > cur.bnd) *pe = kTbInfBits;
      else if (pv < cur.thr) { *pe = kTbInfBits; ready = true; }
      else {
        keep = true; ++carried;
        if (pb < cur.pm) atomicMin((uint32_t*)(g_min + p), pb);
      }
    }
    if (!__any(keep) && lane == 0) A.pflag[cur.pr] = 0;
    const unsigned long long m = __ballot(ready);
    uint32_t base = 0;
    if (lane == 0) base = atomicAdd(&A.bcnt[t], (uint32_t)__popcll(m));
    const bool have_next = k + nwaves < n_pairs;
    const uint32_t pr_after = pairs[min(k + 2u * nwaves, last)];
    const Row nxt = fetch(pr_next, have_next);
    pr_next = pr_after;
    __builtin_amdgcn_sched_barrier(0);
    base = tb::rfl(base);
    if (ready) A.bucket[(size_t)t * A.NP + base + (uint32_t)__popcll(m & ((1ull << lane) - 1ull))] = (uint16_t)p;
    cur = nxt;
  }
  carried = wave_sum(carried);
  if (lane == 0 && carried) A.ctl->n_cand[par ^ 1] = 1u;
}

constexpr uint32_t kTbItemPlans = 16;
__global__ __launch_bounds__(kBlock) void k_tb_items(tb::Args A)
{
  const uint32_t t = blockIdx.x * kBlock + threadIdx.x;
  const int lane = threadIdx.x & 63;
  const uint32_t gran = A.item_plans;
  uint32_t c = 0;
  if (t < A.ntiles) { c = A.bcnt[t]; if (c) A.bcnt[t] = 0u; }
  const uint32_t k = (c + gran - 1u) / gran;
  uint32_t incl = k;
#pragma unroll
  for (int o = 1; o < 64; o <<= 1) { const uint32_t x = __shfl_up(incl, o); if (lane >= o) incl += x; }
  __shared__ uint32_t s_wave[kBlock / 64], s_base;
  const int wave = threadIdx.x >> 6;
  if (lane == 63) s_wave[wave] = incl;
  __syncthreads();
  if (threadIdx.x == 0) {
    uint32_t tot = 0;
#pragma unroll
    for (int w = 0; w < kBlock / 64; ++w) { const uint32_t x = s_wave[w]; s_wave[w] = tot; tot += x; }
    s_base = tot ? atomicAdd(&A.ctl->n_items, tot) : 0u;
  }
  __syncthreads();
  const uint32_t base = s_base + s_wave[wave] + incl - k;
  for (uint32_t q = 0; q < k; ++q) A.items[base + q] = make_uint2(t, (q * gran) | (min(gran, c - q * gran) << 16));
}

__global__ __launch_bounds__(1024) void k_tb_stats(tb::Args A)
{
  __shared__ unsigned long long s_part[16][4];
  unsigned long long acc[4] = { 0ull, 0ull, 0ull, 0ull };
  for (uint32_t w = threadIdx.x; w < A.wstat_slots; w += 1024u)
#pragma unroll
    for (int k = 0; k < 4; ++k) acc[k] += A.wstat[4u * w + k];
#pragma unroll
  for (int k = 0; k < 4; ++k)
#pragma unroll
    for (int o = 32; o > 0; o >>= 1) acc[k] += __shfl_xor(acc[k], o);
  if ((threadIdx.x & 63u) == 0u)
#pragma unroll
    for (int k = 0; k < 4; ++k) s_part[threadIdx.x >> 6][k] = acc[k];
  __syncthreads();
  if (threadIdx.x == 0) {
    unsigned long long t[4] = { 0ull, 0ull, 0ull, 0ull };
    for (int w = 0; w < 16; ++w)
      for (int k = 0; k < 4; ++k) t[k] += s_part[w][k];
    A.ctl->items = t[0]; A.ctl->acts = t[1]; A.ctl->sweeps = t[2]; A.ctl->wakes = t[3];
  }
}

struct TbBlk { uint32_t ya, raw, v[7]; };

#ifdef MNAV_TB_TIMING
__device__ unsigned long long g_tb_timing[8];
#define TB_STAMP(k) do { const unsigned long long now_ = __builtin_readcyclecounter(); tt[k] += now_ - t_last; t_last = now_; } while (0)
#else
#define TB_STAMP(k) do { } while (0)
#endif

constexpr uint32_t kTbQStride = 272;

namespace tb {
__device__ __forceinline__ void ldsw4(uint32_t off, u32x4 v) { *(lds_u32x4_t)(uintptr_t)off = v; }
__device__ __forceinline__ uint32_t wmax4(uint32_t x)
{
  x = max(x, (uint32_t)__shfl_xor((int)x, 16));
  x = max(x, (uint32_t)__shfl_xor((int)x, 32));
  return rfl(x);
}
struct QStream {
  MNAV_GLOBAL const u32x4* st;
  uint32_t last, wr, c; u32x4 c1;
  __device__ __forceinline__ void begin_at(MNAV_GLOBAL const u32x4* first, uint32_t nch, uint32_t stage_q, uint32_t l16)
  {
    st = first + l16;
    last = nch ? nch - 1u : 0u; wr = stage_q + 16u * l16; c = 0;
    ldsw4(wr, st[0]);
    c1 = st[(size_t)min(1u, last) * 16u];
  }
  __device__ __forceinline__ void begin(MNAV_GLOBAL const uint32_t* stream, uint32_t chunk_off, uint32_t nch, uint32_t stage_q, uint32_t l16)
  {
    begin_at((MNAV_GLOBAL const u32x4*)(stream + (size_t)chunk_off * kTbChunk), nch, stage_q, l16);
  }
  __device__ __forceinline__ void advance()
  {
    ldsw4(wr, c1);
    c1 = st[(size_t)min(c + 2u, last) * 16u];
    ++c;
  }
};
}

namespace tb {
template <int Q> __device__ __forceinline__ uint32_t bc(uint32_t d)
{
  return (uint32_t)__builtin_amdgcn_update_dpp(0, (int)d, 0x150 + Q, 0xf, 0xf, true);
}
}

template <bool FIRST>
__device__ __forceinline__ void tb_issue(TbBlk& B, uint32_t D, uint32_t lane4)
{
  B.ya = tb::bc<0>(D) + lane4;
  B.raw = tb::ldsr(B.ya);
  if (FIRST) B.v[0] = tb::ldsr(tb::bc<1>(D) + lane4);
  B.v[1] = tb::ldsr(tb::bc<2>(D) + lane4); B.v[2] = tb::ldsr(tb::bc<3>(D) + lane4);
  B.v[3] = tb::ldsr(tb::bc<4>(D) + lane4); B.v[4] = tb::ldsr(tb::bc<5>(D) + lane4); B.v[5] = tb::ldsr(tb::bc<6>(D) + lane4);
  B.v[6] = tb::ldsr(tb::bc<7>(D) + lane4);
}
template <bool FIRST>
__device__ __forceinline__ uint32_t tb_retire(const TbBlk& B, uint32_t D, uint32_t fwd, bool& ch)
{
  const uint32_t acc0 = B.raw & 0x7fffffffu;
  const uint32_t s0 = FIRST ? B.v[0] : fwd;
  const uint32_t t0 = f2u(fabsf(u2f(s0)) + u2f(tb::bc<8>(D))), t1 = f2u(fabsf(u2f(B.v[1])) + u2f(tb::bc<9>(D)));
  const uint32_t t2 = f2u(fabsf(u2f(B.v[2])) + u2f(tb::bc<10>(D))), t3 = f2u(fabsf(u2f(B.v[3])) + u2f(tb::bc<11>(D)));
  const uint32_t t4 = f2u(fabsf(u2f(B.v[4])) + u2f(tb::bc<12>(D))), t5 = f2u(fabsf(u2f(B.v[5])) + u2f(tb::bc<13>(D)));
  const uint32_t t6 = f2u(fabsf(u2f(B.v[6])) + u2f(tb::bc<14>(D)));
  uint32_t acc = min(min(acc0, t0), t1);
  acc = min(min(acc, t2), t3); acc = min(min(acc, t4), t5); acc = min(acc, t6);
  ch = acc < acc0;
  const uint32_t w = ch ? (acc | kTbDirty) : B.raw;
  tb::ldsw(B.ya, w);
  return w;
}
__device__ __forceinline__ bool tb_chunk(const u32x4& ch4, uint32_t lane4)
{
  TbBlk b0, b1, b2, b3;
  bool c0, c1, c2, c3;
  tb_issue<true>(b0, ch4.x, lane4);
  tb_issue<false>(b1, ch4.y, lane4);
  const uint32_t w0 = tb_retire<true>(b0, ch4.x, 0u, c0);
  tb_issue<false>(b2, ch4.z, lane4);
  const uint32_t w1 = tb_retire<false>(b1, ch4.y, w0, c1);
  tb_issue<false>(b3, ch4.w, lane4);
  const uint32_t w2 = tb_retire<false>(b2, ch4.z, w1, c2);
  (void)tb_retire<false>(b3, ch4.w, w2, c3);
  return c0 | c1 | c2 | c3;
}

#ifndef MNAV_TB_DEPTH
#define MNAV_TB_DEPTH 8
#endif
constexpr int kTbDepth = MNAV_TB_DEPTH;
#ifndef MNAV_TB_ROT
#define MNAV_TB_ROT 2
#endif
constexpr int kTbRot = MNAV_TB_ROT;
template <int T>
__device__ __forceinline__ uint32_t tbq_sweeps(MNAV_GLOBAL const uint32_t* stream, uint32_t sweep_off, uint32_t nch, uint32_t max_nch, uint32_t first_order,
                                               uint32_t l16, uint32_t lane4, bool& overrun)
{
  MNAV_GLOBAL const u32x4* const st0 = (MNAV_GLOBAL const u32x4*)(stream + (size_t)sweep_off * kTbChunk) + l16;
  const uint32_t last = nch ? nch - 1u : 0u;
  uint32_t s_ld = 0, c_ld = 0;
  auto load = [&](u32x4& R) {
    MNAV_GLOBAL const u32x4* const p = st0 + ((size_t)((s_ld + first_order) & 3u) * nch + min(c_ld, last)) * 16u;
    R = *p;
    asm volatile("" ::: "memory");
    if (++c_ld >= max_nch) { c_ld = 0; ++s_ld; }
  };
  unsigned long long any = 0ull;
  uint32_t sweep = 0, c = 0;
  overrun = false;
  bool done = false;
  auto step = [&](u32x4& R) {
    any |= __ballot(tb_chunk(R, lane4));
    load(R);
    if (++c >= max_nch) {
      c = 0; ++sweep;
      if (any == 0ull) done = true;
      else if (sweep >= 16u * T) { overrun = true; done = true; }
      any = 0ull;
    }
  };
  u32x4 R[kTbDepth];
#pragma unroll
  for (int k = 0; k < kTbDepth; ++k) load(R[k]);
  for (;;) {
#pragma unroll
    for (int k = 0; k < kTbRot * kTbDepth; ++k) {
      step(R[k % kTbDepth]);
      if (done) break;
    }
    if (done) break;
  }
  return sweep;
}

template <int T>
__global__ __launch_bounds__(64) void k_tb_solve_q(tb::Args A, int par)
{
#ifdef MNAV_TB_TIMING
  unsigned long long tt[8] = { 0, 0, 0, 0, 0, 0, 0, 0 }, t_last = __builtin_readcyclecounter();
#endif
  __shared__ __attribute__((aligned(16))) uint32_t lds[T * 64 + kTbQStride];
  const int lane = threadIdx.x;
  const uint32_t q = (uint32_t)lane >> 4, l16 = (uint32_t)lane & 15u;
  const uint32_t lds0 = (uint32_t)(uintptr_t)(tb::lds_u32_t)lds;
  const uint32_t lane4 = lds0 + 4u * lane;
  const uint32_t stage_q = lds0 + 4u * (T * 64) + q * kTbQStride;
  const unsigned long long qmask = 0xFFFFull << (16u * q);
  const uint32_t NP = A.NP;
  const uint32_t n_items = A.ctl->n_items;
  MNAV_GLOBAL const uint32_t* const stream = as_global(A.stream);
  uint32_t my_items = 0, my_acts = 0, my_sweeps = 0, my_wakes = 0, my_first = 0;
  bool first_ticket = true;
  for (;;) {
    uint32_t it0 = 4u * blockIdx.x;
    if (!first_ticket) {
      if (lane == 0) it0 = 4u * gridDim.x + atomicAdd(&A.ctl->next_item, 4u);
      it0 = tb::rfl(it0);
    }
    first_ticket = false;
    if (it0 >= n_items) break;
    const u32x2 item = ((MNAV_GLOBAL const u32x2*)as_global(A.items))[min(it0 + q, n_items - 1u)];
    const uint32_t t = item.x, start = item.y & 0xFFFFu, count = (it0 + q < n_items) ? (item.y >> 16) : 0u;
    TbTile W;
    {
      MNAV_GLOBAL const u32x4* hp = (MNAV_GLOBAL const u32x4*)as_global(A.tiles) + 4u * (size_t)t;
      const u32x4 h0 = hp[0], h1 = hp[1], h2 = hp[2];
      W.soff = h0.x; W.sl = h0.y; W.nv = h0.z; W.nh = h0.w;
      W.sweep_off = h1.x; W.sweep_chunks = h1.y; W.pre_off = h1.z; W.pre_chunks = h1.w;
      W.post_off = h2.x; W.post_chunks = h2.y; W.exp_off = h2.z; W.exp_n = h2.w;
    }
    const uint32_t max_sweep = tb::wmax4(W.sweep_chunks), max_pre = tb::wmax4(W.pre_chunks), max_post = tb::wmax4(W.post_chunks),
                   max_exp = tb::wmax4(W.exp_n);
    ++my_items; my_acts += (l16 == 0u) ? count : 0u;
    TB_STAMP(0);
    {
      const bool active = l16 < count;
      const uint32_t p = A.bucket[(size_t)t * NP + start + min(l16, max(count, 1u) - 1u)];
      MNAV_GLOBAL float* sl = as_global(A.D) + ((size_t)W.soff * NP + (size_t)p * W.sl);
      {
        MNAV_GLOBAL const u32x4* s4 = (MNAV_GLOBAL const u32x4*)sl;
        u32x4 v[T / 4];
#pragma unroll
        for (int c = 0; c < T / 4; ++c) v[c] = s4[c];
#pragma unroll
        for (int c = 0; c < T / 4; ++c) {
          tb::ldsw(lane4 + (4 * c + 0) * 256, v[c].x); tb::ldsw(lane4 + (4 * c + 1) * 256, v[c].y);
          tb::ldsw(lane4 + (4 * c + 2) * 256, v[c].z); tb::ldsw(lane4 + (4 * c + 3) * 256, v[c].w);
        }
      }
      MNAV_GLOBAL const u32x4* g4p = (MNAV_GLOBAL const u32x4*)(sl + T);
      uint32_t first_order = 0;
      TB_STAMP(1);
      if (max_pre) {
        tb::QStream S; S.begin(stream, W.pre_off, W.pre_chunks, stage_q, l16);
        u32x4 G = { 0u, 0u, 0u, 0u };
        float gmin = inf_f();
        uint32_t gord = 0;
        for (uint32_t c = 0; c < max_pre; ++c) {
          const bool live = c < W.pre_chunks;
          u32x4 h[kTbBlocksPerChunk], o1[kTbBlocksPerChunk], w2[kTbBlocksPerChunk];
#pragma unroll
          for (int j = 0; j < (int)kTbBlocksPerChunk; ++j) {
            h[j] = tb::ldsr4(stage_q + 64 * j); o1[j] = tb::ldsr4(stage_q + 64 * j + 16); w2[j] = tb::ldsr4(stage_q + 64 * j + 32);
          }
          const u32x4 q3 = tb::ldsr4(stage_q + 48);
          S.advance();
          if (c == 0) G = g4p[live ? q3.x : 0u];
          const u32x4 Gn = g4p[(c + 1u < W.pre_chunks) ? q3.y : 0u];
#pragma unroll
          for (int j = 0; j < (int)kTbBlocksPerChunk; ++j) {
            const uint32_t n = live ? ((h[j].x >> 8) & 7u) : 0u;
            if (n) {
              const uint32_t jj = h[j].x & 3u;
              const float g = u2f(jj == 0 ? G.x : jj == 1 ? G.y : jj == 2 ? G.z : G.w);
              const uint32_t offs[5] = { h[j].y, h[j].z, h[j].w, o1[j].x, o1[j].y };
              const uint32_t ws[5] = { o1[j].z, o1[j].w, w2[j].x, w2[j].y, w2[j].z };
              bool lowered = false;
#pragma unroll
              for (int k = 0; k < (int)kTbGhostEdges; ++k) {
                if ((uint32_t)k < n) {
                  const uint32_t a = offs[k] + lane4;
                  const uint32_t nd = f2u(g + u2f(ws[k]));
                  const uint32_t raw = tb::ldsr(a);
                  const bool low = nd < (raw & 0x7fffffffu);
                  lowered |= low;
                  tb::ldsw(a, low ? (nd | kTbDirty) : raw);
                }
              }
              if (lowered && g < gmin) { gmin = g; gord = (h[j].x >> kTbOrderShift) & 3u; }
            }
          }
          G = Gn;
        }
        const bool votes = active && gmin < inf_f();
        uint32_t bestc = 0;
#pragma unroll
        for (uint32_t o = 0; o < 4; ++o) {
          const uint32_t cn = (uint32_t)__popcll(__ballot(votes && gord == o) & qmask);
          if (cn > bestc) { bestc = cn; first_order = o; }
        }
      }
      TB_STAMP(2);
      bool overrun;
      const uint32_t sweep = max_sweep ? tbq_sweeps<T>(stream, W.sweep_off, W.sweep_chunks, max_sweep, first_order, l16, lane4, overrun) : 1u;
      if (max_sweep && overrun && lane == 0) A.ctl->err = 1u;
      my_sweeps += sweep;
      TB_STAMP(3);
      {
        MNAV_GLOBAL u32x4* s4 = (MNAV_GLOBAL u32x4*)sl;
#pragma unroll
        for (int c = 0; c < T / 4; ++c) {
          u32x4 x;
          x.x = tb::ldsr(lane4 + (4 * c + 0) * 256); x.y = tb::ldsr(lane4 + (4 * c + 1) * 256);
          x.z = tb::ldsr(lane4 + (4 * c + 2) * 256); x.w = tb::ldsr(lane4 + (4 * c + 3) * 256);
          if (active && ((x.x | x.y | x.z | x.w) & kTbDirty)) {
            x.x &= 0x7fffffffu; x.y &= 0x7fffffffu; x.z &= 0x7fffffffu; x.w &= 0x7fffffffu;
            s4[c] = x;
          }
        }
      }
      TB_STAMP(4);
      if (max_post) {
        tb::QStream S; S.begin(stream, W.post_off, W.post_chunks, stage_q, l16);
        u32x4 G = { 0u, 0u, 0u, 0u };
        uint32_t cand = kTbInfBits, best = kTbInfBits;
        MNAV_GLOBAL uint32_t* const pend_p = as_global(A.pend) + p;
        MNAV_GLOBAL uint8_t* const pflag_p = as_global(A.pflag) + (p >> 6);
        MNAV_GLOBAL uint32_t* const pm = as_global(A.marr[par ^ 1]) + p;
        uint32_t t2_1 = 0, best_1 = kTbInfBits, cur_1 = 0, best_2 = kTbInfBits, old_2 = 0;
        bool want_1 = false, did_2 = false;
        uint32_t n_first = 0;
        auto advance = [&](uint32_t t2_new, uint32_t best_new, bool want_new) {
          bool first = false;
          if (did_2) {
            first = old_2 == kTbInfBits;
            if (best_2 < old_2) atomicMin((uint32_t*)pm, best_2);
            ++my_wakes;
          }
          n_first += first ? 1u : 0u;
          did_2 = want_1 && best_1 < cur_1;
          best_2 = best_1;
          if (did_2) { old_2 = atomicMin((uint32_t*)(pend_p + (size_t)t2_1 * NP), best_1); pflag_p[(size_t)t2_1 * A.nblk] = 1; }
          want_1 = want_new; t2_1 = t2_new; best_1 = best_new;
          if (want_new) cur_1 = pend_p[(size_t)t2_new * NP];
        };
        for (uint32_t c = 0; c < max_post; ++c) {
          const bool live = c < W.post_chunks;
          u32x4 h[kTbBlocksPerChunk], o1[kTbBlocksPerChunk], w2[kTbBlocksPerChunk];
#pragma unroll
          for (int j = 0; j < (int)kTbBlocksPerChunk; ++j) {
            h[j] = tb::ldsr4(stage_q + 64 * j); o1[j] = tb::ldsr4(stage_q + 64 * j + 16); w2[j] = tb::ldsr4(stage_q + 64 * j + 32);
          }
          const u32x4 q3 = tb::ldsr4(stage_q + 48);
          S.advance();
          if (c == 0) G = g4p[live ? q3.x : 0u];
          const u32x4 Gn = g4p[(c + 1u < W.post_chunks) ? q3.y : 0u];
#pragma unroll
          for (int j = 0; j < (int)kTbBlocksPerChunk; ++j) {
            const uint32_t hd = live ? h[j].x : 0u, n = (hd >> 8) & 7u;
            if (n) {
              const uint32_t offs[5] = { h[j].y, h[j].z, h[j].w, o1[j].x, o1[j].y };
              const uint32_t ws[5] = { o1[j].z, o1[j].w, w2[j].x, w2[j].y, w2[j].z };
#pragma unroll
              for (int k = 0; k < (int)kTbGhostEdges; ++k)
                if ((uint32_t)k < n) cand = min(cand, f2u(fabsf(u2f(tb::ldsr(offs[k] + lane4))) + u2f(ws[k])));
              if (hd & kTbGhostEnd) {
                const uint32_t jj = hd & 3u;
                const uint32_t g = jj == 0 ? G.x : jj == 1 ? G.y : jj == 2 ? G.z : G.w;
                if (cand < g) best = min(best, cand);
                cand = kTbInfBits;
              }
              if (hd & kTbTileEnd) {
                advance(w2[j].w, best, active && best != kTbInfBits);
                best = kTbInfBits;
              }
            }
          }
          G = Gn;
        }
        advance(0u, kTbInfBits, false);
        advance(0u, kTbInfBits, false);
        my_first |= n_first;
      }
      TB_STAMP(5);
      if (max_exp) {
        tb::QStream S; S.begin_at((MNAV_GLOBAL const u32x4*)as_global(A.exps) + W.exp_off, (W.exp_n + 15u) >> 4, stage_q, l16);
        for (uint32_t k0 = 0; k0 < max_exp; k0 += 16u) {
          u32x4 x[16];
#pragma unroll
          for (int r = 0; r < 16; ++r) x[r] = tb::ldsr4(stage_q + 16 * r);
          S.advance();
#pragma unroll
          for (int r = 0; r < 16; ++r) {
            if (k0 + r < W.exp_n) {
              const uint32_t v = tb::ldsr(x[r].x + lane4);
              if (active && (v & kTbDirty)) as_global(A.D)[(size_t)x[r].y * NP + ((size_t)p * x[r].z + x[r].w)] = u2f(v & 0x7fffffffu);
            }
          }
        }
      }
      TB_STAMP(6);
    }
  }
#ifdef MNAV_TB_TIMING
  if (lane == 0) for (int k = 0; k < 8; ++k) if (tt[k]) atomicAdd(&g_tb_timing[k], tt[k]);
#endif
  my_wakes = wave_sum(my_wakes); my_acts = wave_sum(my_acts);
  if (__any(my_first != 0u) && lane == 0) A.ctl->n_cand[par ^ 1] = 1u;
  if (lane == 0 && my_items && blockIdx.x < A.wstat_slots) {
    unsigned long long* const ws = A.wstat + 4u * blockIdx.x;
    ws[0] += (unsigned long long)my_items; ws[1] += (unsigned long long)my_acts; ws[2] += (unsigned long long)my_sweeps; ws[3] += (unsigned long long)my_wakes;
  }
}

__global__ __launch_bounds__(kWave) void k_tb_path(tb::Args A, const uint32_t* __restrict__ row_ptr, const Nbr* __restrict__ nbr, uint32_t V,
                                                   PlanResult* __restrict__ res, PathRows rows, uint32_t* __restrict__ mismatch)
{
  const uint32_t p = blockIdx.x;
  if (rows.skip(p)) return;
  const int lane = threadIdx.x;
  PlanResult& R = res[p];
  const uint32_t seed = A.seed[p], target = A.target[p];
  const float dt = A.D[tb::slot_addr(A.vaddr[target], A.NP, p)];
  const GoalCut gcut = goal_cut(dt, A.offset, target);
  const float goal_dist = gcut.goal;
  uint32_t code = kSuccess, n = 0, bad = 0;
  if (A.ctl->err || A.ctl->n_cand[0]) code = kInternalError;
  else if (!(dt < inf_f())) code = kNoPathFound;
  else {
    uint32_t* path = rows.row(p);
    const uint32_t cap = rows.capacity(p);
    uint32_t v = target;
    float dv = dt;
    while (v != seed && n <= V) {
      float best_s = inf_f(), best_du = inf_f();
      uint32_t best_u = v;
      const uint32_t beg = row_ptr[v], end = row_ptr[v + 1];
      for (uint32_t i = beg + lane; i < end; i += kWave) {
        const Nbr nb = nbr[i];
        const float du = A.D[tb::slot_addr(A.vaddr[nb.u], A.NP, p)];
        if (!expanded_source(gcut, du, nb.u)) continue;
        const float sm = du + nb.w;
        if (sm < best_s || (sm == best_s && sm < inf_f() && (du < best_du || (du == best_du && nb.u < best_u)))) { best_s = sm; best_du = du; best_u = nb.u; }
      }
#pragma unroll
      for (int o = 1; o < kWave; o <<= 1) {
        const float os = __shfl_xor(best_s, o), odu = __shfl_xor(best_du, o);
        const uint32_t ou = __shfl_xor(best_u, o);
        if (os < best_s || (os == best_s && os < inf_f() && (odu < best_du || (odu == best_du && ou < best_u)))) { best_s = os; best_du = odu; best_u = ou; }
      }
      if (f2u(best_s) != f2u(dv) || best_u == v) { bad = 1; break; }
      v = best_u; dv = best_du;
      if (lane == 0 && n < cap) path[n] = v;
      ++n;
    }
    if (bad || v != seed) code = kInternalError;
    else if (n > cap) code = kPathOverflow;
  }
  if (lane == 0) {
    R.code = code; R.path_len = (code == kSuccess || code == kPathOverflow) ? n : 0;
    R.steps = A.ctl->iters; R.bands = 0; R.armed = (dt < inf_f()) ? 1u : 0u; R.overflow = A.ctl->err;
    R.goal_dist = goal_dist; R.evals = 0; R.shrinks = 0;
    if (bad) atomicAdd(mismatch, 1u);
  }
}

__global__ __launch_bounds__(kWave) void k_tb_vector3(tb::Args A, const uint32_t* __restrict__ row_ptr, const Nbr* __restrict__ nbr,
                                                      const float* __restrict__ xyz, uint32_t p, uint3 vs, float* __restrict__ out)
{
  const int lane = threadIdx.x;
  const uint32_t v = blockIdx.x == 0 ? vs.x : blockIdx.x == 1 ? vs.y : vs.z;
  const float dt = A.D[tb::slot_addr(A.vaddr[A.target[p]], A.NP, p)];
  const GoalCut gcut = goal_cut(dt, A.offset, A.target[p]);
  float best_s = inf_f(), best_du = inf_f();
  uint32_t best_u = v;
  if (v != A.seed[p]) {
    const uint32_t beg = row_ptr[v], end = row_ptr[v + 1];
    for (uint32_t i = beg + lane; i < end; i += kWave) {
      const Nbr nb = nbr[i];
      const float du = A.D[tb::slot_addr(A.vaddr[nb.u], A.NP, p)];
      if (!expanded_source(gcut, du, nb.u)) continue;
      const float sm = du + nb.w;
      if (sm < best_s || (sm == best_s && sm < inf_f() && (du < best_du || (du == best_du && nb.u < best_u)))) { best_s = sm; best_du = du; best_u = nb.u; }
    }
#pragma unroll
    for (int o = 1; o < kWave; o <<= 1) {
      const float os = __shfl_xor(best_s, o), odu = __shfl_xor(best_du, o);
      const uint32_t ou = __shfl_xor(best_u, o);
      if (os < best_s || (os == best_s && os < inf_f() && (odu < best_du || (odu == best_du && ou < best_u)))) { best_s = os; best_du = odu; best_u = ou; }
    }
    if (!(best_s < inf_f())) best_u = v;
  }
  if (lane == 0) {
    float x = 0.f, y = 0.f, z = 0.f;
    if (best_u != v) {
      x = xyz[3 * (size_t)best_u] - xyz[3 * (size_t)v];
      y = xyz[3 * (size_t)best_u + 1] - xyz[3 * (size_t)v + 1];
      z = xyz[3 * (size_t)best_u + 2] - xyz[3 * (size_t)v + 2];
      const float len = sqrtf(x * x + y * y + z * z);
      x = x / len; y = y / len; z = z / len;
    }
    out[3 * blockIdx.x] = x; out[3 * blockIdx.x + 1] = y; out[3 * blockIdx.x + 2] = z;
  }
}

__global__ __launch_bounds__(kBlock) void k_tb_count(tb::Args A, uint32_t T, PlanResult* __restrict__ res)
{
  const uint32_t t = blockIdx.x;
  const int lane = threadIdx.x & 63, wid = threadIdx.x >> 6;
  const TbTile W = A.tiles[t];
  for (uint32_t p = blockIdx.y * (kBlock / 64) + wid; p < A.NP; p += gridDim.y * (kBlock / 64)) {
    const float dt = A.D[tb::slot_addr(A.vaddr[A.target[p]], A.NP, p)];
    const float goal_dist = goal_cut(dt, A.offset, A.target[p]).cut;
    const float* sl = A.D + ((size_t)W.soff * A.NP + (size_t)p * W.sl);
    uint32_t c = 0;
    for (uint32_t i = lane; i < W.nv; i += 64) { const float d = sl[i]; c += (d < inf_f() && d <= goal_dist) ? 1u : 0u; }
    c = wave_sum(c);
    if (lane == 0 && c) atomicAdd(&res[p].settled, (unsigned long long)c);
  }
}

__global__ __launch_bounds__(kBlock) void k_tb_popped(tb::Args A, uint32_t p, uint32_t V, float* __restrict__ out)
{
  const float dt = A.D[tb::slot_addr(A.vaddr[A.target[p]], A.NP, p)];
  const float goal_dist = goal_cut(dt, A.offset, A.target[p]).cut;
  const uint32_t stride = gridDim.x * kBlock;
  for (uint32_t v = blockIdx.x * kBlock + threadIdx.x; v < V; v += stride) {
    const float d = A.D[tb::slot_addr(A.vaddr[v], A.NP, p)];
    out[v] = (d <= goal_dist) ? d : inf_f();
  }
}

__global__ __launch_bounds__(kBlock) void k_popped(const float* __restrict__ dist, uint32_t target, double offset, uint32_t V, float* __restrict__ out)
{
  const float dt = dist[target];
  const float goal_dist = goal_cut(dt, offset, target).cut;
  const uint32_t stride = gridDim.x * kBlock;
  for (uint32_t v = blockIdx.x * kBlock + threadIdx.x; v < V; v += stride) { const float d = dist[v]; out[v] = (d <= goal_dist) ? d : inf_f(); }
}

struct TbTables {
  bool built = false, w_valid = false;
  uint32_t ntiles = 0, max_nh = 0;
  uint64_t S = 0;
  size_t nrec = 0, nexp = 0;
  std::vector<uint32_t> vert_tile;
  DevBuf<uint32_t> d_verts;
  DevBuf<TbTile> d_tiles; DevBuf<uint32_t> d_stream, d_wsrc; DevBuf<TbExp> d_exps;
  DevBuf<uint32_t> d_vstream, d_vwsrc, d_vtile, d_vgroups; DevBuf<TbvExp> d_vexps; size_t nvrec = 0;
  DevBuf<uint2> d_vaddr; DevBuf<uint32_t> d_vert_tile;
  DevBuf<uint16_t> d_fin_src; DevBuf<uint32_t> d_fin_wsrc; DevBuf<float> d_fin_w; DevBuf<TbFinOvf> d_fin_ovf; DevBuf<uint32_t> d_fin_ovf_wsrc; DevBuf<float> d_fin_ovf_w;
  DevBuf<uint32_t> d_ghost_gid, d_fin_order; size_t fin_n = 0, fin_novf = 0; bool fin_w_valid = false; uint32_t max_sl = 0;
};

struct TbBatch {
  uint32_t cap_np = 0;
  DevBuf<float> D; DevBuf<uint32_t> pend; DevBuf<uint8_t> pflag; DevBuf<uint32_t> pairs; DevBuf<uint16_t> bucket; DevBuf<uint32_t> bcnt; DevBuf<uint2> items;
  DevBuf<tb::Ctl> ctl; PinnedBuf<tb::Ctl> h_ctl;
  DevBuf<unsigned long long> wstat; DevBuf<struct FinRec> d_recs;
  DevBuf<uint32_t> marr[2];
  DevBuf<float> thr, bnd; DevBuf<uint32_t> seed, target;
  GraphExec graph[2]; tb::Args graph_args[2]{};
  DevBuf<float> D2; bool d2_clean = false; uint32_t d2_clean_np = 0, d2_wanted_np = 0;
};

struct TbState : TbTables, TbBatch {
  uint32_t T = 120;
  int kernel = 0;
  uint32_t min_batch = 48;
  float band_mult = 2.0f;
  int iters_per_replay = 16, waves_per_cu = 0;
  Stream fill_stream; Event fill_done;
  Event warm_ev[4]; float ms_warm = 0.f, ms_warm_fin = 0.f;
  tb::Ctl last{};
  bool count_pending = false;
};

}

#ifdef MNAV_TB_TIMING
extern "C" int mnav_debug_tb_timing(unsigned long long* out)
{
  if (hipMemcpyFromSymbol(out, HIP_SYMBOL(g_tb_timing), sizeof(unsigned long long) * 8) != hipSuccess) return -1;
  unsigned long long z[8] = { 0, 0, 0, 0, 0, 0, 0, 0 };
  return hipMemcpyToSymbol(HIP_SYMBOL(g_tb_timing), z, sizeof(z)) == hipSuccess ? 0 : -1;
}
#endif
```

### mesh_navigation_amd/csrc/mnav_tb_host.h

```cpp
#pragma once

void tb_free_batch(mnav_ctx* ctx)
{
  TbState& S = ctx->tb;
  if (S.fill_stream) (void)hipStreamSynchronize(S.fill_stream);
  static_cast<TbBatch&>(S) = TbBatch{};
  S.count_pending = false; ctx->tb_args_valid = false;
}

void tb_free(mnav_ctx* ctx)
{
  tb_free_batch(ctx);
  static_cast<TbTables&>(ctx->tb) = TbTables{};
}

int tb_build(mnav_ctx* ctx)
{
  TbState& S = ctx->tb;
  if (S.built) return 0;
  if (opt_set(ctx->opt.tb_tile)) S.T = opt_u32(ctx->opt.tb_tile, S.T);
  if (S.T != 64 && S.T != 96 && S.T != 120 && S.T != 128) S.T = 120;
  HostTopology t;
  t.V = ctx->V; t.E = ctx->E; t.F = ctx->F;
  t.row_ptr = ctx->h_row_ptr; t.nbr_u = ctx->h_nbr_u;
  HostTb H;
  try { H = build_tb(t, ctx->h_xyz.data(), S.T); }
  catch (const std::exception& ex) { ctx->err = ex.what(); return -1; }
  std::vector<uint2> vaddr(ctx->V);
  for (uint32_t v = 0; v < ctx->V; ++v) {
    const TbTile& W = H.tiles[H.vert_tile[v]];
    if (W.sl >= (1u << 24)) { ctx->err = "tile-batch engine: a tile has too many ghosts"; return -1; }
    vaddr[v] = make_uint2(W.soff, (W.sl << 8) | H.vert_local[v]);
  }
  HIPCHK(S.d_tiles.upload(ctx->stream, H.tiles.data(), H.tiles.size()));
  HIPCHK(S.d_stream.upload(ctx->stream, H.stream.data(), H.stream.size()));
  HIPCHK(S.d_wsrc.upload(ctx->stream, H.wsrc.data(), H.wsrc.size()));
  HIPCHK(S.d_exps.upload(ctx->stream, H.exps.data(), H.exps.size()));
  HIPCHK(S.d_vstream.upload(ctx->stream, H.vstream.data(), H.vstream.size()));
  HIPCHK(S.d_vwsrc.upload(ctx->stream, H.vwsrc.data(), H.vwsrc.size()));
  HIPCHK(S.d_vtile.upload(ctx->stream, H.vtile.data(), H.vtile.size()));
  if (H.vgroups.empty()) H.vgroups.push_back(0u);
  HIPCHK(S.d_vgroups.upload(ctx->stream, H.vgroups.data(), H.vgroups.size()));
  HIPCHK(S.d_vexps.upload(ctx->stream, H.vexps.data(), H.vexps.size()));
  HIPCHK(S.d_vaddr.upload(ctx->stream, vaddr.data(), vaddr.size()));
  HIPCHK(S.d_vert_tile.upload(ctx->stream, H.vert_tile.data(), H.vert_tile.size()));
  HIPCHK(S.d_verts.upload(ctx->stream, H.verts.data(), H.verts.size()));
  HIPCHK(S.d_fin_src.upload(ctx->stream, H.fin_src.data(), H.fin_src.size()));
  HIPCHK(S.d_fin_wsrc.upload(ctx->stream, H.fin_wsrc.data(), H.fin_wsrc.size()));
  HIPCHK(S.d_fin_ovf.upload(ctx->stream, H.fin_ovf.data(), H.fin_ovf.size()));
  {
    std::vector<uint32_t> ow(H.fin_ovf.size());
    for (size_t i = 0; i < ow.size(); ++i) ow[i] = H.fin_ovf[i].wsrc;
    HIPCHK(S.d_fin_ovf_wsrc.upload(ctx->stream, ow.data(), ow.size()));
  }
  HIPCHK(S.d_ghost_gid.upload(ctx->stream, H.ghost_gid.data(), H.ghost_gid.size()));
  {
    std::vector<uint32_t> order(H.tiles.size()), key(H.tiles.size(), 0xFFFFFFFFu);
    for (size_t t = 0; t < H.tiles.size(); ++t) {
      order[t] = (uint32_t)t;
      for (uint32_t i = 0; i < H.tiles[t].nv; ++i) key[t] = std::min(key[t], H.verts[H.tiles[t].v0 + i]);
    }
    std::stable_sort(order.begin(), order.end(), [&](uint32_t a, uint32_t b) { return key[a] < key[b]; });
    if (order.empty()) order.push_back(0u);
    HIPCHK(S.d_fin_order.upload(ctx->stream, order.data(), order.size()));
  }
  S.d_fin_w.reset(); S.d_fin_ovf_w.reset();
  S.fin_n = H.fin_src.size(); S.fin_novf = H.fin_ovf.size(); S.fin_w_valid = false; S.max_sl = H.max_sl;
  HIPCHK(S.d_fin_w.alloc(4 * std::max<size_t>(S.fin_n, 1)));
  HIPCHK(S.d_fin_ovf_w.alloc(4 * std::max<size_t>(S.fin_novf, 1)));
  HIPCHK(hipStreamSynchronize(ctx->stream));
  S.nvrec = H.vstream.size();
  S.ntiles = H.ntiles; S.S = H.S; S.nrec = H.stream.size(); S.nexp = H.exps.size(); S.max_nh = H.max_nh;
  S.vert_tile = std::move(H.vert_tile);
  S.built = true; S.w_valid = false;
  if (opt_on(ctx->opt.verbose))
    fprintf(stderr, "[mnav] tile-batch engine: T %u, %u tiles, %.2f slots per vertex, max ghosts %u, %.1f MB of streams + %.1f MB of sweep streams in the V layout\n", S.T, S.ntiles,
            ctx->V ? (double)S.S / ctx->V : 0.0, S.max_nh, (4.0 * S.nrec + 16.0 * S.nexp) / 1e6, 4.0 * S.nvrec / 1e6);
  return 0;
}

int tb_weights(mnav_ctx* ctx)
{
  TbState& S = ctx->tb;
  if (S.w_valid) return 0;
  hipLaunchKernelGGL(k_tb_weights, dim3(4096), dim3(kBlock), 0, ctx->stream, S.nrec, S.d_wsrc, ctx->d_nbr, S.d_stream);
  hipLaunchKernelGGL(k_tb_weights, dim3(4096), dim3(kBlock), 0, ctx->stream, S.nvrec, S.d_vwsrc, ctx->d_nbr, S.d_vstream);
  HIPCHK(hipGetLastError());
  S.w_valid = true; S.fin_w_valid = false;
  return 0;
}

int tb_fin_weights(mnav_ctx* ctx)
{
  TbState& S = ctx->tb;
  if (S.fin_w_valid) return 0;
  hipLaunchKernelGGL(k_tb_fin_weights, dim3(4096), dim3(kBlock), 0, ctx->stream, S.fin_n, S.d_fin_wsrc, ctx->d_nbr, S.d_fin_w);
  if (S.fin_novf) hipLaunchKernelGGL(k_tb_fin_weights, dim3(64), dim3(kBlock), 0, ctx->stream, S.fin_novf, S.d_fin_ovf_wsrc, ctx->d_nbr, S.d_fin_ovf_w);
  HIPCHK(hipGetLastError());
  S.fin_w_valid = true;
  return 0;
}

int tb_ensure_batch(mnav_ctx* ctx, uint32_t np)
{
  TbState& S = ctx->tb;
  if (np <= S.cap_np) return 0;
  tb_free_batch(ctx);
  const size_t nt = S.ntiles ? S.ntiles : 1, pairs = nt * (size_t)np;
  HIPCHK(S.D.alloc(4 * (size_t)S.S * np + 64));
  if (8 * (size_t)S.S * np <= ((size_t)96 << 30) && !opt_on(ctx->opt.tb_no_prefill)) {
    if (S.D2.alloc(4 * (size_t)S.S * np + 64) != hipSuccess) (void)hipGetLastError();
    if (S.D2 && !S.fill_stream) { HIPCHK(hipStreamCreateWithFlags(S.fill_stream.out(), hipStreamNonBlocking)); HIPCHK(hipEventCreateWithFlags(S.fill_done.out(), hipEventDisableTiming)); }
  }
  HIPCHK(S.pend.alloc(4 * pairs + 64));
  HIPCHK(S.pflag.alloc(nt * (((size_t)np + 63) / 64) + 64));
  HIPCHK(S.pairs.alloc(4 * (nt * (((size_t)np + 63) / 64) + 64)));
  HIPCHK(S.bucket.alloc(2 * pairs + 64));
  HIPCHK(S.bcnt.alloc(4 * nt));
  HIPCHK(S.items.alloc(8 * (nt + pairs / kTbItemPlans + 64)));
  HIPCHK(S.ctl.alloc(sizeof(tb::Ctl)));
  HIPCHK(S.wstat.alloc(32 * (size_t)kTbStatSlots));
  HIPCHK(S.h_ctl.alloc(sizeof(tb::Ctl)));
  for (int k = 0; k < 2; ++k) HIPCHK(S.marr[k].alloc(4 * (size_t)np));
  HIPCHK(S.thr.alloc(4 * (size_t)np)); HIPCHK(S.bnd.alloc(4 * (size_t)np));
  HIPCHK(S.seed.alloc(4 * (size_t)np)); HIPCHK(S.target.alloc(4 * (size_t)np));
  HIPCHK(S.d_recs.alloc(sizeof(FinRec) * (size_t)np));
  S.cap_np = np;
  return 0;
}

int tb_fill(mnav_ctx* ctx, void* p, size_t bytes, uint32_t v)
{
  const size_t n16 = (bytes + 15) / 16;
  uint32_t g = (uint32_t)std::min<size_t>((n16 + kBlock - 1) / kBlock, 256 * 32);
  if (g < 1) g = 1;
  hipLaunchKernelGGL(k_tb_fill, dim3(g), dim3(kBlock), 0, ctx->stream, (u32x4*)p, n16, v);
  HIPCHK(hipGetLastError());
  return 0;
}

int tb_launch_iterations(mnav_ctx* ctx, const tb::Args& A, int count, uint32_t waves)
{
  const uint32_t gp = (A.NP + kBlock - 1) / kBlock;
  for (int j = 0; j < count; ++j) {
    const int par = j & 1;
    hipLaunchKernelGGL(k_tb_plan, dim3(gp), dim3(kBlock), 0, ctx->stream, A, par);
    hipLaunchKernelGGL(k_tb_pairs, dim3((A.n_flag16 + kBlock * kTbPairUnits - 1) / (kBlock * kTbPairUnits)), dim3(kBlock), 0, ctx->stream, A);
    hipLaunchKernelGGL(k_tb_scan, dim3(kTbScanWaves / (kBlock / 64)), dim3(kBlock), 0, ctx->stream, A, par);
    hipLaunchKernelGGL(k_tb_items, dim3((A.ntiles + kBlock - 1) / kBlock), dim3(kBlock), 0, ctx->stream, A);
    if (ctx->tb.kernel == 1) hipLaunchKernelGGL((k_tbv_solve<120>), dim3(waves), dim3(64), 0, ctx->stream, A, ctx->tb.d_vtile, ctx->tb.d_vstream, ctx->tb.d_vgroups, ctx->tb.d_vexps, par);
    else if (ctx->tb.T == 64) hipLaunchKernelGGL((k_tb_solve_q<64>), dim3(waves), dim3(64), 0, ctx->stream, A, par);
    else if (ctx->tb.T == 96) hipLaunchKernelGGL((k_tb_solve_q<96>), dim3(waves), dim3(64), 0, ctx->stream, A, par);
    else if (ctx->tb.T == 120) hipLaunchKernelGGL((k_tb_solve_q<120>), dim3(waves), dim3(64), 0, ctx->stream, A, par);
    else hipLaunchKernelGGL((k_tb_solve_q<128>), dim3(waves), dim3(64), 0, ctx->stream, A, par);
  }
  hipLaunchKernelGGL(k_tb_stats, dim3(1), dim3(1024), 0, ctx->stream, A);
  HIPCHK(hipGetLastError());
  return 0;
}

int tb_fields(mnav_ctx* ctx, uint32_t n, const std::vector<PlanIn>& in, double offset, const tb::Args& A)
{
  TbState& S = ctx->tb;
  if (ensure_slots(ctx, n, false, false, ctx->want_vec)) return -1;
  if (tb_fin_weights(ctx)) return -1;
  std::vector<Plan> hp(n);
  std::vector<float*> vecs(n);
  for (uint32_t i = 0; i < n; ++i) {
    Slot& s = ctx->slots[i];
    Plan& P = hp[i];
    memset(&P, 0, sizeof(P));
    P.planner = kPlannerDijkstra; P.V = ctx->V;
    P.row_ptr = ctx->d_row_ptr.get(); P.nbr = ctx->d_nbr.get(); P.crn_ptr = ctx->d_crn_ptr.get(); P.crn = ctx->d_crn.get(); P.blocked = ctx->d_blocked.get();
    P.dist = s.dist.get(); P.pred = s.pred.get(); P.cap = ctx->V; P.ctl = s.ctl; P.cnt = s.cnt.get();
    P.offset = offset; P.max_steps = ctx->max_steps;
    for (int k = 0; k < 3; ++k) { P.seed[k] = in[i].seed[k]; P.target[k] = in[i].target[k]; P.seed_d[k] = 0.f; P.seed_expands[k] = 1; P.target_expands[k] = 1; }
    P.seed_face = kNone;
    vecs[i] = s.vecmap;
  }
  HIPCHK(hipMemcpyAsync(ctx->d_plans, hp.data(), sizeof(Plan) * n, hipMemcpyHostToDevice, ctx->stream));
  HIPCHK(hipMemcpyAsync(ctx->d_vecptrs, vecs.data(), sizeof(float*) * n, hipMemcpyHostToDevice, ctx->stream));
  HIPCHK(hipStreamSynchronize(ctx->stream));
  FinTb F{};
  F.src = S.d_fin_src; F.w = S.d_fin_w; F.ovf = S.d_fin_ovf; F.ovf_w = S.d_fin_ovf_w; F.verts = S.d_verts; F.ghost_gid = S.d_ghost_gid; F.order = S.d_fin_order;
  F.xyz = ctx->d_xyz; F.vecmaps = ctx->want_vec ? ctx->d_vecptrs : nullptr;
  F.plans = ctx->d_plans; F.res = ctx->d_res; F.mismatch = ctx->d_mismatch; F.recs = S.d_recs;
  const uint32_t groups = (S.ntiles + kFinWaves - 1u) / kFinWaves;
#ifndef MNAV_FIN_PPW
#define MNAV_FIN_PPW 64u
#endif
  F.plans_per_wave = MNAV_FIN_PPW; F.tiles_per_xcd = (groups + 7u) / 8u; F.max_sl = S.max_sl;
  hipLaunchKernelGGL(k_tb_fin_plans, dim3((n + kBlock - 1) / kBlock), dim3(kBlock), 0, ctx->stream, A, ctx->d_plans, F.vecmaps, S.d_recs);
  const uint32_t npg = (n + F.plans_per_wave - 1u) / F.plans_per_wave;
  const size_t lds = 4 * (size_t)fin_lds_words(S.max_sl, F.vecmaps != nullptr) * kFinWaves;
  const dim3 grid(8u * F.tiles_per_xcd * npg);
  if (S.T == 64) hipLaunchKernelGGL((k_tb_finalize<64>), grid, dim3(64 * kFinWaves), lds, ctx->stream, A, F);
  else if (S.T == 96) hipLaunchKernelGGL((k_tb_finalize<96>), grid, dim3(64 * kFinWaves), lds, ctx->stream, A, F);
  else if (S.T == 120) hipLaunchKernelGGL((k_tb_finalize<120>), grid, dim3(64 * kFinWaves), lds, ctx->stream, A, F);
  else hipLaunchKernelGGL((k_tb_finalize<128>), grid, dim3(64 * kFinWaves), lds, ctx->stream, A, F);
  HIPCHK(hipGetLastError());
  return 0;
}

int tb_clean_other(mnav_ctx* ctx)
{
  TbState& S = ctx->tb;
  if (!S.D2 || !S.fill_stream || S.d2_wanted_np == 0u || S.d2_clean) return 0;
  const uint32_t n = S.d2_wanted_np;
  S.d2_wanted_np = 0u;
  const size_t n16 = (4 * (size_t)S.S * n + 15) / 16;
  const uint32_t g = (uint32_t)std::max<size_t>(std::min<size_t>((n16 + kBlock - 1) / kBlock, 256 * 32), 1);
  hipLaunchKernelGGL(k_tb_fill, dim3(g), dim3(kBlock), 0, S.fill_stream, (u32x4*)S.D2.get(), n16, kTbInfBits);
  HIPCHK(hipEventRecord(S.fill_done, S.fill_stream));
  S.d2_clean = true; S.d2_clean_np = n;
  return 0;
}

struct TbWarmIn { const uint32_t* d_level; const float* const* d_dist; ReplanCnt* d_cnt; };

int run_dijkstra_tb(mnav_ctx* ctx, uint32_t n, const std::vector<PlanIn>& in, double offset, const TbWarmIn* warm = nullptr)
{
  TbState& S = ctx->tb;
  if (tb_build(ctx)) return -1;
  if (tb_weights(ctx)) return -1;
  if (n > 65535u) { ctx->err = "tile-batch engine: more than 65535 plans in one batch"; return -1; }
  if (tb_ensure_batch(ctx, n)) return -1;
  if (ensure_plan_tables(ctx, n)) return -1;
  if (ensure_paths(ctx, n)) return -1;
  if (!ctx->d_mismatch) HIPCHK(ctx->d_mismatch.alloc(4));
  std::vector<uint32_t> seeds(n), targets(n);
  for (uint32_t i = 0; i < n; ++i) { seeds[i] = in[i].seed[0]; targets[i] = in[i].target[0]; }
  HIPCHK(hipMemcpyAsync(S.seed, seeds.data(), 4 * (size_t)n, hipMemcpyHostToDevice, ctx->stream));
  HIPCHK(hipMemcpyAsync(S.target, targets.data(), 4 * (size_t)n, hipMemcpyHostToDevice, ctx->stream));
  HIPCHK(hipMemsetAsync(ctx->d_res, 0, sizeof(PlanResult) * n, ctx->stream));
  HIPCHK(hipMemsetAsync(ctx->d_mismatch, 0, 4, ctx->stream));
  tb::Args A{};
  A.tiles = S.d_tiles; A.stream = S.d_stream; A.exps = S.d_exps; A.D = S.D; A.pend = S.pend; A.pflag = S.pflag; A.nblk = (n + 63u) / 64u; A.NP = n; A.ntiles = S.ntiles;
  A.bucket = S.bucket; A.bcnt = S.bcnt; A.items = S.items; A.ctl = S.ctl; A.wstat = S.wstat; A.wstat_slots = kTbStatSlots;
  A.pairs = S.pairs; A.n_flag16 = (uint32_t)(((size_t)S.ntiles * A.nblk + 15u) / 16u);
  tb_div_magic(A.nblk, &A.nblk_magic, &A.nblk_shift);
  if ((size_t)S.ntiles * A.nblk >= (1ull << 31)) { ctx->err = "tile-batch engine: flag matrix beyond 2^31 entries"; return -1; }
  A.marr[0] = S.marr[0]; A.marr[1] = S.marr[1];
  A.thr = S.thr; A.bnd = S.bnd; A.seed = S.seed; A.target = S.target; A.vaddr = S.d_vaddr; A.vert_tile = S.d_vert_tile;
  A.offset = offset;
  const bool v_fits = S.T == 120 && S.max_nh <= kTbvGhostRows;
  const double density = (double)n / std::sqrt((double)std::max(S.ntiles, 1u));
  S.kernel = (v_fits && density >= 8.0) ? 1 : 0;
  if (opt_set(ctx->opt.tb_kernel)) S.kernel = (opt_u32(ctx->opt.tb_kernel, 0u) == 1u && v_fits) ? 1 : 0;
  A.item_plans = S.kernel == 1 ? 64u : kTbItemPlans;
  {
    const float band_mult = (S.kernel == 1 && density < 40.0) ? 4.0f : S.band_mult;
    float band = (ctx->delta_auto / 3.0f) * std::sqrt((float)S.T) * band_mult;
    if (opt_set(ctx->opt.tb_band_mult)) band = (ctx->delta_auto / 3.0f) * std::sqrt((float)S.T) * (float)ctx->opt.tb_band_mult;
    if (ctx->tile_band_user > 0.f) band = ctx->tile_band_user;
    A.band = band;
  }
  HIPCHK(hipEventRecord(ctx->ev[1], ctx->stream));
  if (!warm) {
    bool prefilled = false;
    if (S.D2 && S.d2_clean && S.d2_clean_np >= n) {
      std::swap(S.D, S.D2); A.D = S.D;
      HIPCHK(hipStreamWaitEvent(ctx->stream, S.fill_done, 0));
      prefilled = true;
    }
    S.d2_clean = false;
    if (!prefilled && tb_fill(ctx, S.D, 4 * (size_t)S.S * n, kTbInfBits)) return -1;
    if (tb_fill(ctx, S.pend, 4 * (size_t)S.ntiles * n, kTbInfBits)) return -1;
  }
  HIPCHK(hipMemsetAsync(S.pflag, 0, (size_t)(S.ntiles ? S.ntiles : 1) * ((n + 63u) / 64u) + 64u, ctx->stream));
  if (tb_fill(ctx, S.marr[0], 4 * (size_t)n, kTbInfBits)) return -1;
  if (tb_fill(ctx, S.marr[1], 4 * (size_t)n, kTbInfBits)) return -1;
  HIPCHK(hipMemsetAsync(S.ctl, 0, sizeof(tb::Ctl), ctx->stream));
  HIPCHK(hipMemsetAsync(S.wstat, 0, 32 * (size_t)kTbStatSlots, ctx->stream));
  HIPCHK(hipMemsetAsync(S.bcnt, 0, 4 * (size_t)(S.ntiles ? S.ntiles : 1), ctx->stream));
  if (warm) {
    if (!S.warm_ev[0]) for (auto& e : S.warm_ev) HIPCHK(hipEventCreate(e.out()));
    HIPCHK(hipMemsetAsync(warm->d_cnt, 0, sizeof(ReplanCnt) * (size_t)n, ctx->stream));
    TbWarm Wm{};
    Wm.level = warm->d_level; Wm.dist = warm->d_dist; Wm.cnt = warm->d_cnt;
    Wm.verts = S.d_verts; Wm.ghost_gid = S.d_ghost_gid; Wm.order = S.d_fin_order; Wm.T = S.T;
    const size_t groups = (size_t)std::max(S.ntiles, 1u) * ((n + 63u) / 64u);
    if (groups >= (1ull << 31)) { ctx->err = "tile-batch engine: warm start beyond 2^31 workgroups"; return -1; }
    HIPCHK(hipEventRecord(S.warm_ev[0], ctx->stream));
    if (S.ntiles) hipLaunchKernelGGL(k_tb_warm, dim3((uint32_t)groups), dim3(kWarmBlock), 0, ctx->stream, A, Wm);
    HIPCHK(hipEventRecord(S.warm_ev[1], ctx->stream));
  } else
  hipLaunchKernelGGL(k_tb_seed, dim3((n + kBlock - 1) / kBlock), dim3(kBlock), 0, ctx->stream, A);
  HIPCHK(hipGetLastError());
  HIPCHK(hipEventRecord(ctx->ev[2], ctx->stream));
  if (!warm || !S.d2_clean) S.d2_wanted_np = S.D2 ? n : 0u;

  int ncu = 256;
  (void)hipDeviceGetAttribute(&ncu, hipDeviceAttributeMultiprocessorCount, ctx->device);
  uint32_t per_cu = (uint32_t)((160u * 1024u) / (S.T * 256u + kTbQStride * 4u));
  if (S.kernel == 1) per_cu = 8u;
  if (opt_set(ctx->opt.tb_waves_per_cu)) S.waves_per_cu = (int)ctx->opt.tb_waves_per_cu;
  if (S.waves_per_cu > 0) per_cu = (uint32_t)S.waves_per_cu;
  const uint32_t waves = per_cu * (uint32_t)ncu;
  const int chunk = S.iters_per_replay & ~1;
  int gi = 0;
  for (int k = 0; k < 2; ++k) if (S.graph[k] && memcmp(&S.graph_args[k], &A, sizeof(A)) == 0) gi = k + 2;
  if (ctx->use_graph && gi < 2) {
    gi = (S.graph[0] && S.graph_args[0].D != A.D) ? 1 : 0;
    S.graph[gi].reset();
    hipGraph_t g = nullptr;
    HIPCHK(hipStreamBeginCapture(ctx->stream, hipStreamCaptureModeThreadLocal));
    const int rc = tb_launch_iterations(ctx, A, chunk, waves);
    const hipError_t e = hipStreamEndCapture(ctx->stream, &g);
    if (rc != 0 || e != hipSuccess) { ctx->err = "graph capture failed"; return -1; }
    HIPCHK(hipGraphInstantiate(S.graph[gi].out(), g, nullptr, nullptr, 0));
    (void)hipGraphDestroy(g);
    memcpy(&S.graph_args[gi], &A, sizeof(A));
  } else gi -= 2;
  int rc = 0;
  uint32_t iters = 0;
  const auto t_start = std::chrono::steady_clock::now();
  HIPCHK(hipEventRecord(ctx->evc[0], ctx->stream));
  for (;;) {
    if (std::chrono::duration<double>(std::chrono::steady_clock::now() - t_start).count() > ctx->max_wall_s) {
      ctx->err = "tile-batch iterations exceeded the wall-clock guard"; return -1;
    }
    if (ctx->use_graph) HIPCHK(hipGraphLaunch(S.graph[gi], ctx->stream));
    else if (tb_launch_iterations(ctx, A, chunk, waves)) return -1;
    iters += (uint32_t)chunk;
    HIPCHK(hipMemcpyAsync(S.h_ctl, S.ctl, sizeof(tb::Ctl), hipMemcpyDeviceToHost, ctx->stream));
    HIPCHK(hipStreamSynchronize(ctx->stream));
    if (S.h_ctl->err) { ctx->err = "tile-batch engine: sweep cap hit"; return -1; }
    if (S.h_ctl->n_cand[0] == 0u) break;
    if (ctx->cancel.load(std::memory_order_relaxed)) { rc = 1; break; }
    if (iters > ctx->max_steps) { ctx->err = "tile-batch engine: iteration cap hit"; return -1; }
  }
  HIPCHK(hipEventRecord(ctx->evc[1], ctx->stream));
  if (rc == 0 && !ctx->lazy_paths) {
    if (warm) HIPCHK(hipEventRecord(S.warm_ev[2], ctx->stream));
    if (tb_fields(ctx, n, in, offset, A)) return -1;
    if (warm) HIPCHK(hipEventRecord(S.warm_ev[3], ctx->stream));
  }
  HIPCHK(hipEventRecord(ctx->ev[3], ctx->stream));
  HIPCHK(hipEventSynchronize(ctx->evc[1]));
  ctx->ms_chunks = ev_ms(ctx->evc[0], ctx->evc[1]);
  S.last = *S.h_ctl;
  if (warm && rc == 0) {
    HIPCHK(hipEventSynchronize(S.warm_ev[3]));
    S.ms_warm = ev_ms(S.warm_ev[0], S.warm_ev[1]); S.ms_warm_fin = ev_ms(S.warm_ev[2], S.warm_ev[3]);
  }
  ctx->stats.launches = 1;
  ctx->tb_args = A; ctx->tb_args_valid = (rc == 0);
  if (opt_on(ctx->opt.trace))
    fprintf(stderr, "[mnav] tile-batch: %u iterations, %llu activations (%.1f per item), %llu items, %.2f sweeps per item, %llu wakes\n", S.h_ctl->iters,
            S.h_ctl->acts, S.h_ctl->items ? (double)S.h_ctl->acts / S.h_ctl->items : 0.0, S.h_ctl->items,
            S.h_ctl->items ? (double)S.h_ctl->sweeps / S.h_ctl->items : 0.0, S.h_ctl->wakes);
  return rc;
}
```

Before: 42580.

## Pack paths on device, async mismatch check, and per-tile scheduler replacing pair scan

Computes path offsets with a device scan and packs paths before the first sync, avoiding a host round trip and extra H2D copies. The mismatch counter is read asynchronously into pinned memory instead of a blocking hipMemcpy. In the tile-batch engine, the flag-compaction and pair-scan kernels are replaced by a per-tile wave scheduler that keeps several blocks in flight and writes per-tile bucket counts without atomics. Atomic-min contention is spread over 64 carry copies that k_tb_plan then reduces. This adds a 64-way reduction each iteration and extra memory, and the fill stream is now ordered after the call.

```diff
diff --git a/mesh_navigation_amd/csrc/mnav.hip b/mesh_navigation_amd/csrc/mnav.hip
--- a/mesh_navigation_amd/csrc/mnav.hip
+++ b/mesh_navigation_amd/csrc/mnav.hip
@@ -143,7 +143,8 @@
   DevBuf<float*> d_vecptrs;
   DevBuf<uint32_t> d_paths; size_t paths_words = 0; uint32_t path_stride = 0;
   DevBuf<uint32_t> d_over; DevBuf<unsigned long long> d_over_off; DevBuf<uint32_t> d_over_cap;
-  DevBuf<uint32_t> d_pack; PinnedBuf<uint32_t> h_pack; DevBuf<uint32_t> d_pack_meta; size_t pack_words = 0, pack_meta_n = 0;
+  DevBuf<uint32_t> d_pack; PinnedBuf<uint32_t> h_pack; DevBuf<uint32_t> d_pack_meta; size_t pack_words = 0, h_pack_words = 0, pack_meta_n = 0;
+  PinnedBuf<uint32_t> h_mism;
   PinnedBuf<Ctl> h_ctl;
   uint32_t infl_exact_bands = 0;
   DevBuf<float> d_seed_pos; uint32_t seed_pos_cap = 1;
@@ -1307,8 +1308,31 @@
   if (want_vecmap && n_vec && !(engine == 5 && !ctx->lazy_paths))
     hipLaunchKernelGGL(k_vecmap_dijkstra, dim3(gc ? gc : 1, n_vec), dim3(kBlock), 0, ctx->stream, d_plans, ctx->d_xyz, sub ? sub->vecptrs : ctx->d_vecptrs.get());
   (void)hipEventRecord(ctx->ev[5], ctx->stream);
+  const bool pack = path_out && path_cap;
+  auto ensure_pack = [&](size_t words) {
+    if (ctx->pack_words < words) {
+      ctx->d_pack.reset(); ctx->pack_words = 0;
+      if (ctx->d_pack.alloc(4 * words) != hipSuccess) return false;
+      ctx->pack_words = words;
+    }
+    if (ctx->pack_meta_n < 2 * (size_t)m) {
+      ctx->pack_meta_n = 0;
+      if (ctx->d_pack_meta.alloc(4 * 2 * (size_t)m) != hipSuccess) return false;
+      ctx->pack_meta_n = 2 * (size_t)m;
+    }
+    return true;
+  };
+  if (pack) {
+    if (!ensure_pack((size_t)m * (ctx->path_stride ? ctx->path_stride : 1u))) { ctx->err = "path buffers: out of memory"; return -1; }
+    hipLaunchKernelGGL(k_pack_offsets, dim3(1), dim3(1024), 0, ctx->stream, d_res, m, ctx->d_pack_meta, ctx->d_pack_meta + m);
+    hipLaunchKernelGGL(k_pack_paths, dim3(m), dim3(kBlock), 0, ctx->stream, rows1, rows2, ctx->d_pack_meta, ctx->d_pack_meta + m, ctx->d_pack);
+  }
+  const bool check_mism = ctx->last_engine != 1;
+  if (check_mism && !ctx->h_mism && ctx->h_mism.alloc(4) != hipSuccess) { ctx->err = "result download failed"; return -1; }
   if (hipMemcpyAsync(ctx->h_res, d_res, sizeof(PlanResult) * m, hipMemcpyDeviceToHost, ctx->stream) != hipSuccess ||
+      (check_mism && hipMemcpyAsync(ctx->h_mism, ctx->d_mismatch, 4, hipMemcpyDeviceToHost, ctx->stream) != hipSuccess) ||
       hipStreamSynchronize(ctx->stream) != hipSuccess) { ctx->err = "result download failed"; return -1; }
+  bool repack = false;
   {
     size_t over_words = 0;
     std::vector<unsigned long long> ooff(m, 0ull); std::vector<uint32_t> ocap(m, 0u);
@@ -1326,16 +1350,15 @@
       else if (ctx->lazy_paths) hipLaunchKernelGGL(k_path_lazy, dim3(m), dim3(kWave), 0, ctx->stream, ctx->d_plans, ctx->d_tplans, ctx->d_res, rows2, ctx->d_mismatch);
       else hipLaunchKernelGGL(k_finish<kPlannerDijkstra>, dim3(m), dim3(64), 0, ctx->stream, d_plans, d_res, rows2);
       if (hipMemcpyAsync(ctx->h_res, d_res, sizeof(PlanResult) * m, hipMemcpyDeviceToHost, ctx->stream) != hipSuccess ||
+          (check_mism && hipMemcpyAsync(ctx->h_mism, ctx->d_mismatch, 4, hipMemcpyDeviceToHost, ctx->stream) != hipSuccess) ||
           hipStreamSynchronize(ctx->stream) != hipSuccess) { ctx->err = "result download failed"; return -1; }
       for (uint32_t k = 0; k < m; ++k) ctx->h_res[k].settled = keep[k].settled;
-    }
-  }
-  if (ctx->last_engine != 1) {
-    uint32_t mism = 0;
-    if (hipMemcpy(&mism, ctx->d_mismatch, 4, hipMemcpyDeviceToHost) != hipSuccess || mism != 0) {
-      ctx->err = "tiled SSSP did not reach its fixed point (" + std::to_string(mism) + " vertices)";
-      return -1;
-    }
+      repack = true;
+    }
+  }
+  if (check_mism && *ctx->h_mism != 0u) {
+    ctx->err = "tiled SSSP did not reach its fixed point (" + std::to_string(*ctx->h_mism) + " vertices)";
+    return -1;
   }
   MTRACE("results downloaded");
   std::vector<uint32_t> offs(m + 1, 0), lens(m, 0);
@@ -1344,26 +1367,25 @@
     offs[k + 1] = offs[k] + lens[k];
   }
   const size_t total = offs[m];
-  if (total && path_out && path_cap) {
-    if (ctx->pack_words < total) {
-      ctx->d_pack.reset(); ctx->h_pack.reset(); ctx->pack_words = 0;
+  if (total && pack) {
+    if (ctx->h_pack_words < total) {
+      ctx->h_pack.reset(); ctx->h_pack_words = 0;
       const size_t want = total + total / 4 + 1024;
-      if (ctx->d_pack.alloc(4 * want) != hipSuccess || ctx->h_pack.alloc(4 * want) != hipSuccess)
-        { ctx->err = "path buffers: out of memory"; return -1; }
-      ctx->pack_words = want;
-    }
-    if (ctx->pack_meta_n < 2 * (size_t)m) {
-      ctx->pack_meta_n = 0;
-      if (ctx->d_pack_meta.alloc(4 * 2 * (size_t)m) != hipSuccess) { ctx->err = "path buffers: out of memory"; return -1; }
-      ctx->pack_meta_n = 2 * (size_t)m;
-    }
-    if (hipMemcpyAsync(ctx->d_pack_meta, offs.data(), 4 * (size_t)m, hipMemcpyHostToDevice, ctx->stream) != hipSuccess ||
-        hipMemcpyAsync(ctx->d_pack_meta + m, lens.data(), 4 * (size_t)m, hipMemcpyHostToDevice, ctx->stream) != hipSuccess)
-      { ctx->err = "path download failed"; return -1; }
-    hipLaunchKernelGGL(k_pack_paths, dim3(m), dim3(kBlock), 0, ctx->stream, rows1, rows2, ctx->d_pack_meta, ctx->d_pack_meta + m, ctx->d_pack);
-    if (hipMemcpyAsync(ctx->h_pack, ctx->d_pack, 4 * total, hipMemcpyDeviceToHost, ctx->stream) != hipSuccess ||
-        hipStreamSynchronize(ctx->stream) != hipSuccess) { ctx->err = "path download failed"; return -1; }
-  }
+      if (ctx->h_pack.alloc(4 * want) != hipSuccess) { ctx->err = "path buffers: out of memory"; return -1; }
+      ctx->h_pack_words = want;
+    }
+    if (repack) {
+      if (!ensure_pack(total)) { ctx->err = "path buffers: out of memory"; return -1; }
+      if (hipMemcpyAsync(ctx->d_pack_meta, offs.data(), 4 * (size_t)m, hipMemcpyHostToDevice, ctx->stream) != hipSuccess ||
+          hipMemcpyAsync(ctx->d_pack_meta + m, lens.data(), 4 * (size_t)m, hipMemcpyHostToDevice, ctx->stream) != hipSuccess)
+        { ctx->err = "path download failed"; return -1; }
+      hipLaunchKernelGGL(k_pack_paths, dim3(m), dim3(kBlock), 0, ctx->stream, rows1, rows2, ctx->d_pack_meta, ctx->d_pack_meta + m, ctx->d_pack);
+    }
+    if (hipMemcpyAsync(ctx->h_pack, ctx->d_pack, 4 * total, hipMemcpyDeviceToHost, ctx->stream) != hipSuccess) { ctx->err = "path download failed"; return -1; }
+  }
+  const bool field_downloads = dist_out || pred_out || (vecmap_out && want_vecmap);
+  if (engine == 5 && !field_downloads && tb_clean_other(ctx)) return -1;
+  if (total && pack && hipStreamSynchronize(ctx->stream) != hipSuccess) { ctx->err = "path download failed"; return -1; }
   MTRACE("paths downloaded");
   for (uint32_t k = 0; k < m; ++k) {
     const uint32_t i = map[k];
diff --git a/mesh_navigation_amd/csrc/mnav_plan_kernels.h b/mesh_navigation_amd/csrc/mnav_plan_kernels.h
--- a/mesh_navigation_amd/csrc/mnav_plan_kernels.h
+++ b/mesh_navigation_amd/csrc/mnav_plan_kernels.h
@@ -170,6 +170,29 @@
   for (uint32_t q = threadIdx.x; q < len; q += kBlock) dst[q] = src[len - 1 - q];
 }
 
+__global__ __launch_bounds__(1024) void k_pack_offsets(const PlanResult* __restrict__ res, uint32_t m, uint32_t* __restrict__ offs, uint32_t* __restrict__ lens)
+{
+  __shared__ uint32_t s_wave[16], s_carry;
+  const uint32_t lane = threadIdx.x & 63u, wave = threadIdx.x >> 6;
+  if (threadIdx.x == 0) s_carry = 0u;
+  __syncthreads();
+  for (uint32_t base = 0; base < m; base += 1024u) {
+    const uint32_t k = base + threadIdx.x;
+    const uint32_t len = (k < m && res[k].code == kSuccess) ? res[k].path_len : 0u;
+    uint32_t incl = len;
+#pragma unroll
+    for (int o = 1; o < 64; o <<= 1) { const uint32_t x = __shfl_up(incl, o); if (lane >= (uint32_t)o) incl += x; }
+    if (lane == 63u) s_wave[wave] = incl;
+    __syncthreads();
+    uint32_t before = s_carry;
+    for (uint32_t w = 0; w < wave; ++w) before += s_wave[w];
+    if (k < m) { offs[k] = before + incl - len; lens[k] = len; }
+    __syncthreads();
+    if (threadIdx.x == 1023u) s_carry = before + incl;
+    __syncthreads();
+  }
+}
+
 __global__ __launch_bounds__(kBlock) void k_count_goal(const Plan* __restrict__ plans, PlanResult* __restrict__ res)
 {
   const Plan& P = plans[blockIdx.y];
diff --git a/mesh_navigation_amd/csrc/mnav_tb.h b/mesh_navigation_amd/csrc/mnav_tb.h
--- a/mesh_navigation_amd/csrc/mnav_tb.h
+++ b/mesh_navigation_amd/csrc/mnav_tb.h
@@ -23,7 +23,6 @@
   unsigned long long sweeps;
   unsigned long long items;
   unsigned long long wakes;
-  uint32_t n_pairs, pad_;
 };
 
 struct Args {
@@ -31,13 +30,12 @@
   float* D; uint32_t* pend; uint32_t NP, ntiles;
   uint16_t* bucket; uint32_t* bcnt; uint2* items; Ctl* ctl;
   uint32_t* marr[2];
+  uint32_t* mcarry;
   float* thr; float* bnd;
   const uint32_t* seed; const uint32_t* target;
   const uint2* vaddr; const uint32_t* vert_tile;
   double offset; float band;
   uint8_t* pflag; uint32_t nblk;
-  uint32_t* pairs; uint32_t n_flag16;
-  uint32_t nblk_magic, nblk_shift;
   unsigned long long* wstat; uint32_t wstat_slots;
   uint32_t item_plans;
 };
@@ -53,11 +51,6 @@
 __device__ __forceinline__ u32x4 ldsr4(uint32_t off) { return *(lds_u32x4_t)(uintptr_t)off; }
 
 __device__ __forceinline__ uint32_t rfl(uint32_t x) { return (uint32_t)__builtin_amdgcn_readfirstlane((int)x); }
-
-__device__ __forceinline__ uint32_t div_by_magic(uint32_t n, uint32_t d, uint32_t magic, uint32_t shift)
-{
-  return d <= 1u ? n : (__umulhi(n, magic) >> shift);
-}
 
 }
 
@@ -97,13 +90,24 @@
   A.ctl->n_cand[0] = 1u;
 }
 
+constexpr uint32_t kTbMinCopies = 64;
 __global__ __launch_bounds__(kBlock) void k_tb_plan(tb::Args A, int par)
 {
   const uint32_t p = blockIdx.x * kBlock + threadIdx.x;
-  if (p == 0) { A.ctl->n_cand[par ^ 1] = 0u; A.ctl->next_item = 0u; A.ctl->n_items = 0u; A.ctl->n_pairs = 0u; A.ctl->iters += 1u; }
+  if (p == 0) { A.ctl->n_cand[par ^ 1] = 0u; A.ctl->next_item = 0u; A.ctl->n_items = 0u; A.ctl->iters += 1u; }
   if (p >= A.NP) return;
-  const uint32_t mb = A.marr[par][p];
+  uint32_t mb = A.marr[par][p];
   A.marr[par ^ 1][p] = kTbInfBits;
+  {
+    uint32_t x[kTbMinCopies];
+#pragma unroll
+    for (uint32_t c = 0; c < kTbMinCopies; ++c) x[c] = A.mcarry[(size_t)c * A.NP + p];
+#pragma unroll
+    for (uint32_t c = 0; c < kTbMinCopies; ++c) {
+      mb = min(mb, x[c]);
+      if (x[c] != kTbInfBits) A.mcarry[(size_t)c * A.NP + p] = kTbInfBits;
+    }
+  }
   const float m = u2f(mb);
   const float dt = A.D[tb::slot_addr(A.vaddr[A.target[p]], A.NP, p)];
   const float bound = (float)((double)dt + fmax(A.offset, 0.0));
@@ -114,106 +118,99 @@
   A.bnd[p] = bound;
 }
 
-constexpr uint32_t kTbPairUnits = 4;
-__global__ __launch_bounds__(kBlock) void k_tb_pairs(tb::Args A)
-{
-  __shared__ uint32_t s_wave[kBlock / 64], s_base;
-  const int lane = threadIdx.x & 63, wave = threadIdx.x >> 6;
-  const uint32_t i0 = (blockIdx.x * kBlock + threadIdx.x) * kTbPairUnits;
-  u32x4 f[kTbPairUnits];
+constexpr uint32_t kTbStatSlots = 16384;
+constexpr uint32_t kTbSchedTiles = kBlock / 64;
+#ifndef MNAV_TB_SCHED_DEPTH
+#define MNAV_TB_SCHED_DEPTH 4
+#endif
+constexpr uint32_t kTbSchedDepth = MNAV_TB_SCHED_DEPTH;
+__global__ __launch_bounds__(kBlock) void k_tb_sched(tb::Args A, int par)
+{
+  const uint32_t lane = threadIdx.x & 63u;
+  const uint32_t t = tb::rfl(blockIdx.x * kTbSchedTiles + (threadIdx.x >> 6));
+  if (t >= A.ntiles) return;
+  const uint32_t nblk = A.nblk, NP = A.NP;
+  MNAV_GLOBAL uint8_t* const g_flag = as_global(A.pflag) + (size_t)t * nblk;
+  auto flags = [&](uint32_t c) { const uint32_t i = c * 64u + lane; return i < nblk ? (uint32_t)g_flag[i] : 0u; };
+  const uint32_t f0 = flags(0u), f1 = flags(1u);
+  unsigned long long m = __ballot(f0 != 0u), m_next = __ballot(f1 != 0u);
   uint32_t c = 0;
-#pragma unroll
-  for (uint32_t u = 0; u < kTbPairUnits; ++u) {
-    f[u] = u32x4{ 0u, 0u, 0u, 0u };
-    if (i0 + u < A.n_flag16) f[u] = ((MNAV_GLOBAL const u32x4*)as_global(A.pflag))[i0 + u];
-    const uint32_t w[4] = { f[u].x, f[u].y, f[u].z, f[u].w };
-#pragma unroll
-    for (int k = 0; k < 4; ++k)
-#pragma unroll
-      for (int b = 0; b < 4; ++b) c += ((w[k] >> (8 * b)) & 0xFFu) ? 1u : 0u;
-  }
-  uint32_t incl = c;
-#pragma unroll
-  for (int o = 1; o < 64; o <<= 1) { const uint32_t x = __shfl_up(incl, o); if (lane >= o) incl += x; }
-  if (lane == 63) s_wave[wave] = incl;
-  __syncthreads();
-  if (threadIdx.x == 0) {
-    uint32_t tot = 0;
-#pragma unroll
-    for (int w = 0; w < kBlock / 64; ++w) { const uint32_t x = s_wave[w]; s_wave[w] = tot; tot += x; }
-    s_base = tot ? atomicAdd(&A.ctl->n_pairs, tot) : 0u;
-  }
-  __syncthreads();
-  uint32_t base = s_base + s_wave[wave] + incl - c;
-  if (c) {
-#pragma unroll
-    for (uint32_t u = 0; u < kTbPairUnits; ++u) {
-      const uint32_t w[4] = { f[u].x, f[u].y, f[u].z, f[u].w };
-#pragma unroll
-      for (int k = 0; k < 4; ++k)
-#pragma unroll
-        for (int b = 0; b < 4; ++b)
-          if ((w[k] >> (8 * b)) & 0xFFu) A.pairs[base++] = 16u * (i0 + u) + 4u * k + b;
-    }
-  }
-}
-
-constexpr uint32_t kTbStatSlots = 16384;
-constexpr uint32_t kTbScanWaves = 8192;
-__global__ __launch_bounds__(kBlock) void k_tb_scan(tb::Args A, int par)
-{
-  const int lane = threadIdx.x & 63;
-  const uint32_t wave = blockIdx.x * (kBlock / 64) + (threadIdx.x >> 6), nwaves = gridDim.x * (kBlock / 64);
-  const uint32_t n_pairs = A.ctl->n_pairs;
-  if (wave >= n_pairs) return;
-  MNAV_GLOBAL const uint32_t* const pairs = as_global(A.pairs);
+  auto next_block = [&]() -> uint32_t {
+    while (m == 0ull) {
+      if ((c + 1u) * 64u >= nblk) return kNone;
+      ++c; m = m_next; m_next = __ballot(flags(c + 1u) != 0u);
+    }
+    const uint32_t b = c * 64u + (uint32_t)__builtin_ctzll(m);
+    m &= m - 1ull;
+    return b;
+  };
+  const uint32_t b_first = next_block();
+  if (b_first == kNone) return;
   MNAV_GLOBAL const float* const g_thr = as_global(A.thr);
   MNAV_GLOBAL const float* const g_bnd = as_global(A.bnd);
-  MNAV_GLOBAL uint32_t* const g_pend = as_global(A.pend);
-  MNAV_GLOBAL uint32_t* const g_min = as_global(A.marr[par ^ 1]);
-  uint32_t carried = 0;
-  struct Row { uint32_t pr, t, p, pb, pm; float thr, bnd; bool live; };
-  auto fetch = [&](uint32_t pr, bool have) {
-    Row r; r.pr = pr;
-    const uint32_t t = tb::div_by_magic(pr, A.nblk, A.nblk_magic, A.nblk_shift), p = (pr - t * A.nblk) * 64u + (uint32_t)lane;
-    r.live = have && t < A.ntiles && p < A.NP;
-    r.t = r.live ? t : 0u; r.p = r.live ? p : 0u;
-    r.pb = g_pend[(size_t)r.t * A.NP + r.p]; r.thr = g_thr[r.p]; r.bnd = g_bnd[r.p]; r.pm = g_min[r.p];
+  MNAV_GLOBAL uint32_t* const g_pend = as_global(A.pend) + (size_t)t * NP;
+  MNAV_GLOBAL uint16_t* const g_bucket = as_global(A.bucket) + (size_t)t * NP;
+  MNAV_GLOBAL uint32_t* const g_min = as_global(A.mcarry) + (size_t)(t % kTbMinCopies) * NP;
+  struct Row { uint32_t p, pb, pm; float thr, bnd; bool live; };
+  auto fetch = [&](uint32_t b) {
+    Row r;
+    const uint32_t p = (b != kNone ? b : 0u) * 64u + lane;
+    r.live = b != kNone && p < NP;
+    r.p = r.live ? p : 0u;
+    r.pb = g_pend[r.p]; r.thr = g_thr[r.p]; r.bnd = g_bnd[r.p]; r.pm = g_min[r.p];
     return r;
   };
-  uint32_t k = wave;
-  const uint32_t last = n_pairs - 1u;
-  uint32_t pr_next = pairs[min(k + nwaves, last)];
-  Row cur = fetch(pairs[k], true);
-  for (; k < n_pairs; k += nwaves) {
-    asm volatile("" :: "v"(cur.pb), "v"(cur.thr), "v"(cur.bnd), "v"(cur.pm));
-    const uint32_t t = cur.t, p = cur.p, pb = cur.pb;
-    MNAV_GLOBAL uint32_t* const pe = g_pend + ((size_t)t * A.NP + p);
-    bool ready = false, keep = false;
-    if (cur.live && pb != kTbInfBits) {
-      const float pv = u2f(pb);
-      if (pv > cur.bnd) *pe = kTbInfBits;
-      else if (pv < cur.thr) { *pe = kTbInfBits; ready = true; }
-      else {
-        keep = true; ++carried;
-        if (pb < cur.pm) atomicMin((uint32_t*)(g_min + p), pb);
+  const unsigned long long below = (1ull << lane) - 1ull;
+  uint32_t count = 0;
+  bool carried = false;
+  constexpr int K = (int)kTbSchedDepth;
+  uint32_t b_cur[K];
+  Row cur[K];
+  b_cur[0] = b_first;
+#pragma unroll
+  for (int k = 1; k < K; ++k) b_cur[k] = next_block();
+#pragma unroll
+  for (int k = 0; k < K; ++k) cur[k] = fetch(b_cur[k]);
+  for (;;) {
+    uint32_t b_next[K];
+    Row nxt[K];
+#pragma unroll
+    for (int k = 0; k < K; ++k) b_next[k] = next_block();
+#pragma unroll
+    for (int k = 0; k < K; ++k) nxt[k] = fetch(b_next[k]);
+    __builtin_amdgcn_sched_barrier(0);
+#pragma unroll
+    for (int k = 0; k < K; ++k)
+      asm volatile("" :: "v"(cur[k].pb), "v"(cur[k].thr), "v"(cur[k].bnd), "v"(cur[k].pm));
+#pragma unroll
+    for (int k = 0; k < K; ++k) {
+      if (b_cur[k] == kNone) break;
+      const uint32_t p = cur[k].p, pb = cur[k].pb;
+      bool ready = false, keep = false;
+      if (cur[k].live && pb != kTbInfBits) {
+        const float pv = u2f(pb);
+        if (pv > cur[k].bnd) g_pend[p] = kTbInfBits;
+        else if (pv < cur[k].thr) { g_pend[p] = kTbInfBits; ready = true; }
+        else {
+          keep = true;
+          if (pb < cur[k].pm) atomicMin((uint32_t*)(g_min + p), pb);
+        }
       }
-    }
-    if (!__any(keep) && lane == 0) A.pflag[cur.pr] = 0;
-    const unsigned long long m = __ballot(ready);
-    uint32_t base = 0;
-    if (lane == 0) base = atomicAdd(&A.bcnt[t], (uint32_t)__popcll(m));
-    const bool have_next = k + nwaves < n_pairs;
-    const uint32_t pr_after = pairs[min(k + 2u * nwaves, last)];
-    const Row nxt = fetch(pr_next, have_next);
-    pr_next = pr_after;
-    __builtin_amdgcn_sched_barrier(0);
-    base = tb::rfl(base);
-    if (ready) A.bucket[(size_t)t * A.NP + base + (uint32_t)__popcll(m & ((1ull << lane) - 1ull))] = (uint16_t)p;
-    cur = nxt;
-  }
-  carried = wave_sum(carried);
-  if (lane == 0 && carried) A.ctl->n_cand[par ^ 1] = 1u;
+      const bool any_keep = __any(keep);
+      carried |= any_keep;
+      if (!any_keep && lane == 0u) g_flag[b_cur[k]] = 0;
+      const unsigned long long rm = __ballot(ready);
+      if (ready) g_bucket[count + (uint32_t)__popcll(rm & below)] = (uint16_t)p;
+      count += (uint32_t)__popcll(rm);
+    }
+    if (b_next[0] == kNone) break;
+#pragma unroll
+    for (int k = 0; k < K; ++k) { cur[k] = nxt[k]; b_cur[k] = b_next[k]; }
+  }
+  if (lane == 0u) {
+    if (count) A.bcnt[t] = count;
+    if (carried) A.ctl->n_cand[par ^ 1] = 1u;
+  }
 }
 
 constexpr uint32_t kTbItemPlans = 16;
@@ -767,7 +764,7 @@
 
 struct TbBatch {
   uint32_t cap_np = 0;
-  DevBuf<float> D; DevBuf<uint32_t> pend; DevBuf<uint8_t> pflag; DevBuf<uint32_t> pairs; DevBuf<uint16_t> bucket; DevBuf<uint32_t> bcnt; DevBuf<uint2> items;
+  DevBuf<float> D; DevBuf<uint32_t> pend; DevBuf<uint32_t> mcarry; DevBuf<uint8_t> pflag; DevBuf<uint16_t> bucket; DevBuf<uint32_t> bcnt; DevBuf<uint2> items;
   DevBuf<tb::Ctl> ctl; PinnedBuf<tb::Ctl> h_ctl;
   DevBuf<unsigned long long> wstat; DevBuf<struct FinRec> d_recs;
   DevBuf<uint32_t> marr[2];
@@ -782,7 +779,7 @@
   uint32_t min_batch = 48;
   float band_mult = 2.0f;
   int iters_per_replay = 16, waves_per_cu = 0;
-  Stream fill_stream; Event fill_done;
+  Stream fill_stream; Event fill_done, call_done;
   Event warm_ev[4]; float ms_warm = 0.f, ms_warm_fin = 0.f;
   tb::Ctl last{};
   bool count_pending = false;
diff --git a/mesh_navigation_amd/csrc/mnav_tb_host.h b/mesh_navigation_amd/csrc/mnav_tb_host.h
--- a/mesh_navigation_amd/csrc/mnav_tb_host.h
+++ b/mesh_navigation_amd/csrc/mnav_tb_host.h
@@ -110,11 +110,10 @@
   HIPCHK(S.D.alloc(4 * (size_t)S.S * np + 64));
   if (8 * (size_t)S.S * np <= ((size_t)96 << 30) && !opt_on(ctx->opt.tb_no_prefill)) {
     if (S.D2.alloc(4 * (size_t)S.S * np + 64) != hipSuccess) (void)hipGetLastError();
-    if (S.D2 && !S.fill_stream) { HIPCHK(hipStreamCreateWithFlags(S.fill_stream.out(), hipStreamNonBlocking)); HIPCHK(hipEventCreateWithFlags(S.fill_done.out(), hipEventDisableTiming)); }
+    if (S.D2 && !S.fill_stream) { HIPCHK(hipStreamCreateWithFlags(S.fill_stream.out(), hipStreamNonBlocking)); HIPCHK(hipEventCreateWithFlags(S.fill_done.out(), hipEventDisableTiming)); HIPCHK(hipEventCreateWithFlags(S.call_done.out(), hipEventDisableTiming)); }
   }
   HIPCHK(S.pend.alloc(4 * pairs + 64));
   HIPCHK(S.pflag.alloc(nt * (((size_t)np + 63) / 64) + 64));
-  HIPCHK(S.pairs.alloc(4 * (nt * (((size_t)np + 63) / 64) + 64)));
   HIPCHK(S.bucket.alloc(2 * pairs + 64));
   HIPCHK(S.bcnt.alloc(4 * nt));
   HIPCHK(S.items.alloc(8 * (nt + pairs / kTbItemPlans + 64)));
@@ -122,6 +121,7 @@
   HIPCHK(S.wstat.alloc(32 * (size_t)kTbStatSlots));
   HIPCHK(S.h_ctl.alloc(sizeof(tb::Ctl)));
   for (int k = 0; k < 2; ++k) HIPCHK(S.marr[k].alloc(4 * (size_t)np));
+  HIPCHK(S.mcarry.alloc(4 * (size_t)kTbMinCopies * np + 64));
   HIPCHK(S.thr.alloc(4 * (size_t)np)); HIPCHK(S.bnd.alloc(4 * (size_t)np));
   HIPCHK(S.seed.alloc(4 * (size_t)np)); HIPCHK(S.target.alloc(4 * (size_t)np));
   HIPCHK(S.d_recs.alloc(sizeof(FinRec) * (size_t)np));
@@ -145,8 +145,7 @@
   for (int j = 0; j < count; ++j) {
     const int par = j & 1;
     hipLaunchKernelGGL(k_tb_plan, dim3(gp), dim3(kBlock), 0, ctx->stream, A, par);
-    hipLaunchKernelGGL(k_tb_pairs, dim3((A.n_flag16 + kBlock * kTbPairUnits - 1) / (kBlock * kTbPairUnits)), dim3(kBlock), 0, ctx->stream, A);
-    hipLaunchKernelGGL(k_tb_scan, dim3(kTbScanWaves / (kBlock / 64)), dim3(kBlock), 0, ctx->stream, A, par);
+    hipLaunchKernelGGL(k_tb_sched, dim3(std::max((A.ntiles + kTbSchedTiles - 1) / kTbSchedTiles, 1u)), dim3(kBlock), 0, ctx->stream, A, par);
     hipLaunchKernelGGL(k_tb_items, dim3((A.ntiles + kBlock - 1) / kBlock), dim3(kBlock), 0, ctx->stream, A);
     if (ctx->tb.kernel == 1) hipLaunchKernelGGL((k_tbv_solve<120>), dim3(waves), dim3(64), 0, ctx->stream, A, ctx->tb.d_vtile, ctx->tb.d_vstream, ctx->tb.d_vgroups, ctx->tb.d_vexps, par);
     else if (ctx->tb.T == 64) hipLaunchKernelGGL((k_tb_solve_q<64>), dim3(waves), dim3(64), 0, ctx->stream, A, par);
@@ -210,6 +209,8 @@
   S.d2_wanted_np = 0u;
   const size_t n16 = (4 * (size_t)S.S * n + 15) / 16;
   const uint32_t g = (uint32_t)std::max<size_t>(std::min<size_t>((n16 + kBlock - 1) / kBlock, 256 * 32), 1);
+  HIPCHK(hipEventRecord(S.call_done, ctx->stream));
+  HIPCHK(hipStreamWaitEvent(S.fill_stream, S.call_done, 0));
   hipLaunchKernelGGL(k_tb_fill, dim3(g), dim3(kBlock), 0, S.fill_stream, (u32x4*)S.D2.get(), n16, kTbInfBits);
   HIPCHK(hipEventRecord(S.fill_done, S.fill_stream));
   S.d2_clean = true; S.d2_clean_np = n;
@@ -237,10 +238,7 @@
   tb::Args A{};
   A.tiles = S.d_tiles; A.stream = S.d_stream; A.exps = S.d_exps; A.D = S.D; A.pend = S.pend; A.pflag = S.pflag; A.nblk = (n + 63u) / 64u; A.NP = n; A.ntiles = S.ntiles;
   A.bucket = S.bucket; A.bcnt = S.bcnt; A.items = S.items; A.ctl = S.ctl; A.wstat = S.wstat; A.wstat_slots = kTbStatSlots;
-  A.pairs = S.pairs; A.n_flag16 = (uint32_t)(((size_t)S.ntiles * A.nblk + 15u) / 16u);
-  tb_div_magic(A.nblk, &A.nblk_magic, &A.nblk_shift);
-  if ((size_t)S.ntiles * A.nblk >= (1ull << 31)) { ctx->err = "tile-batch engine: flag matrix beyond 2^31 entries"; return -1; }
-  A.marr[0] = S.marr[0]; A.marr[1] = S.marr[1];
+  A.marr[0] = S.marr[0]; A.marr[1] = S.marr[1]; A.mcarry = S.mcarry;
   A.thr = S.thr; A.bnd = S.bnd; A.seed = S.seed; A.target = S.target; A.vaddr = S.d_vaddr; A.vert_tile = S.d_vert_tile;
   A.offset = offset;
   const bool v_fits = S.T == 120 && S.max_nh <= kTbvGhostRows;
@@ -270,6 +268,7 @@
   HIPCHK(hipMemsetAsync(S.pflag, 0, (size_t)(S.ntiles ? S.ntiles : 1) * ((n + 63u) / 64u) + 64u, ctx->stream));
   if (tb_fill(ctx, S.marr[0], 4 * (size_t)n, kTbInfBits)) return -1;
   if (tb_fill(ctx, S.marr[1], 4 * (size_t)n, kTbInfBits)) return -1;
+  if (tb_fill(ctx, S.mcarry, 4 * (size_t)kTbMinCopies * n, kTbInfBits)) return -1;
   HIPCHK(hipMemsetAsync(S.ctl, 0, sizeof(tb::Ctl), ctx->stream));
   HIPCHK(hipMemsetAsync(S.wstat, 0, 32 * (size_t)kTbStatSlots, ctx->stream));
   HIPCHK(hipMemsetAsync(S.bcnt, 0, 4 * (size_t)(S.ntiles ? S.ntiles : 1), ctx->stream));
@@ -296,7 +295,7 @@
   if (S.kernel == 1) per_cu = 8u;
   if (opt_set(ctx->opt.tb_waves_per_cu)) S.waves_per_cu = (int)ctx->opt.tb_waves_per_cu;
   if (S.waves_per_cu > 0) per_cu = (uint32_t)S.waves_per_cu;
-  const uint32_t waves = per_cu * (uint32_t)ncu;
+  const uint32_t waves = std::min(per_cu * (uint32_t)ncu, kTbStatSlots);
   const int chunk = S.iters_per_replay & ~1;
   int gi = 0;
   for (int k = 0; k < 2; ++k) if (S.graph[k] && memcmp(&S.graph_args[k], &A, sizeof(A)) == 0) gi = k + 2;
```

Result: faster. 44310, median of 6 (+4.0%).
